# qiutang98/chord

Hardware: AMD Instinct MI355X
Metric: Gtri/s into 4K 64-bit visbuffer (higher is better)
Workload: dtype f32+u64; 1 GPU; street_4k_hzb; scene_triangles_lod0=2799616, objects=352, hzb=True, cull=flat, parallelism=single

## Files before the change

### chord_amd/csrc/kernels_raster.hip

```cpp

#include "device_layer.h"
#include "device_math.h"

#include <algorithm>
#include <cstdlib>
#include <cstring>
#include <type_traits>

namespace chord {

#define GUARD_BAND 1024.0f
#define LDS_VERTS 256
#define TILE CHORD_TILE
#define TILE_SHIFT CHORD_TILE_SHIFT
#define TPITCH (TILE + 1)
#define SMALL_AREA 256
#define TC_STRIDE CHORD_TILECOUNT_STRIDE
#define TC_BLOCKS 1u
#define TC_TICKET 2u
#ifndef CHORD_MASKED_FUSED
#define CHORD_MASKED_FUSED 1
#endif
#define TC_MASKED 3u

struct RasterParams {
    const uint32_t* count; const ChordDrawCmd* cmds;
    uint32_t cmdCap;
    uint32_t* leftCount; ChordDrawCmd* leftCmds;
    const DObjFrame* objFrame; const DObjStatic* objStatic;
    const DMeshlet* meshlets; const uint32_t* meshletData; const float* positions;
    const DMaterial* materials; const uint8_t* texAlpha; const float* texcoords;
    unsigned long long* vis;
    float* depthOut;
    float W, H; int32_t Wi, Hi;
    ShardInfo shard;
    TriRec* tris; uint32_t triCap;
    TriRecC* trisC; uint32_t triCapC;
    uint32_t* tileCount; uint32_t* tileBins; uint32_t binCap; uint32_t tilesX, tilesY;
    uint32_t* binPool; uint32_t binPoolChunks; uint32_t* binPoolCount;
    unsigned long long* binChunkTab; uint32_t binStamp; uint32_t binMaxChunks;
    unsigned long long* blockPool; uint32_t blockCap;
    uint32_t blockForce;
    ClipTri* clipTris; uint32_t clipTriCap; uint32_t pass;
    uint32_t* largeList; uint32_t largeCap;
    DeviceCounters* counters;
    uint2* tileOrder;
    unsigned long long* tileSlabs;
    uint32_t hzbFused;
    ChordHZBDesc hzbDesc;
    uint16_t* hzbMinA;
    uint16_t* hzbMinB; uint16_t* hzbMaxB;
    uint16_t* hzbExA;
    uint16_t* hzbExB;
    uint32_t* tileRange;
    unsigned long long* tileClocks;
    unsigned long long* tilePhase;
    uint32_t depthOnly, depthClamp;
    float biasConst, biasSlope;
    uint32_t clearTiles;
    uint32_t* binHint;
    uint32_t* countHint;
    uint32_t slotHot;
    uint32_t* hotTiles;
    uint32_t tileSlots;
    uint32_t tileSplitMin, tileSliceLen;
    uint2* tileOrderNext;
    uint32_t orderAll;
    uint32_t orderKept;
    uint32_t* heavyHint;
    uint32_t debug;
};
#define ABL(p, flag) (RASTER_ABLATION && ((p).debug & (flag)) != 0u)
#define DBG_NO_PIXELS   1u
#define DBG_NO_BIN      2u
#define DBG_TILE_CLOCKS 16u
#define DBG_NO_OUT      128u
#define DBG_NO_HZB      256u
#define DBG_SETUP_CLOCKS 512u
#define DBG_NO_VIS_STORE 1024u
#define DBG_NO_SPLIT    2048u
#define DBG_NO_TINY     32u
#define DBG_TILE_EXIT   64u
#define DBG_NO_ENTRY    8192u
#define DBG_NO_BATCH    16384u
#define DBG_NO_UNITS    4096u
#define DBG_SKIP_LIGHT  1048576u
#define DBG_SKIP_HEAVY  2097152u

template <typename T>
__device__ __forceinline__ T scalar_load(const T* ptr)
{
    return *reinterpret_cast<const __attribute__((address_space(4))) T*>(reinterpret_cast<uintptr_t>(ptr));
}
__device__ __forceinline__ const RasterParams* kernel_args()
{
    unsigned long long kp = (unsigned long long)__builtin_amdgcn_kernarg_segment_ptr();
    asm volatile("" : "+s"(kp));
    return reinterpret_cast<const RasterParams*>(kp);
}

__device__ __forceinline__ uint32_t mbcnt64(unsigned long long m) { return __builtin_amdgcn_mbcnt_hi((uint32_t)(m >> 32), __builtin_amdgcn_mbcnt_lo((uint32_t)m, 0u)); }
__device__ __forceinline__ int32_t bcast(int32_t v, int src) { return __builtin_amdgcn_readlane(v, src); }
__device__ __forceinline__ uint32_t bcast(uint32_t v, int src) { return (uint32_t)__builtin_amdgcn_readlane((int)v, src); }
__device__ __forceinline__ float bcast(float v, int src) { return __int_as_float(__builtin_amdgcn_readlane(__float_as_int(v), src)); }

__device__ __forceinline__ bool owns_tile(const ShardInfo& s, int32_t tx, int32_t ty)
{
    if (s.ranks <= 1) return true;
    return shard_owns_tile(s, (uint32_t)tx, (uint32_t)ty);
}
__device__ __forceinline__ bool owns_rect(const ShardInfo& s, int32_t px0, int32_t py0, int32_t px1, int32_t py1)
{
    if (s.ranks <= 1) return true;
    return shard_owns_any_tile(s, (uint32_t)px0 >> TILE_SHIFT, (uint32_t)py0 >> TILE_SHIFT, (uint32_t)px1 >> TILE_SHIFT, (uint32_t)py1 >> TILE_SHIFT);
}

__device__ __forceinline__ bool in_fast_volume_xy(const f4& h)
{
    return h.w > 0.0f && (GUARD_BAND * h.w + h.x) >= 0.0f && (GUARD_BAND * h.w - h.x) >= 0.0f &&
           (GUARD_BAND * h.w + h.y) >= 0.0f && (GUARD_BAND * h.w - h.y) >= 0.0f;
}

__device__ __forceinline__ bool in_fast_volume(const f4& h)
{
    return h.w > 0.0f && (h.w - h.z) >= 0.0f && h.z >= 0.0f &&
           (GUARD_BAND * h.w + h.x) >= 0.0f && (GUARD_BAND * h.w - h.x) >= 0.0f &&
           (GUARD_BAND * h.w + h.y) >= 0.0f && (GUARD_BAND * h.w - h.y) >= 0.0f;
}

struct TriSetup {
    int32_t X[3], Y[3];
    float d0, e1, e2, invA;
    int32_t px0, py0, px1, py1;
    int64_t area;
    int32_t s;
    uint32_t payload;
};

__device__ __forceinline__ bool narrow_extent(const TriSetup& ts)
{
    const int32_t extX = max(ts.X[0], max(ts.X[1], ts.X[2])) - min(ts.X[0], min(ts.X[1], ts.X[2]));
    const int32_t extY = max(ts.Y[0], max(ts.Y[1], ts.Y[2])) - min(ts.Y[0], min(ts.Y[1], ts.Y[2]));
    return extX <= (1 << 14) && extY <= (1 << 14);
}

__device__ __forceinline__ bool fits_compact(const TriSetup& ts)
{
    return narrow_extent(ts);
}

__device__ __forceinline__ void write_record_c(TriRecC* dst, const TriSetup& ts, const float d[3])
{
    TriRecC r;
    r.X0 = ts.X[0]; r.Y0 = ts.Y[0];
    r.dX1 = (int16_t)(ts.X[1] - ts.X[0]); r.dY1 = (int16_t)(ts.Y[1] - ts.Y[0]);
    r.dX2 = (int16_t)(ts.X[2] - ts.X[0]); r.dY2 = (int16_t)(ts.Y[2] - ts.Y[0]);
    r.d[0] = d[0]; r.d[1] = d[1]; r.d[2] = d[2];
    r.payload = ts.payload;
    *dst = r;
}

__device__ __forceinline__ bool tri_setup(TriSetup& ts, bool twoSided, int32_t Wi, int32_t Hi)
{
    const int32_t dx1 = ts.X[1] - ts.X[0], dy1 = ts.Y[1] - ts.Y[0], dx2 = ts.X[2] - ts.X[0], dy2 = ts.Y[2] - ts.Y[0];
    int64_t area2;
    const bool small = (uint32_t)(dx1 + 32767) < 65535u && (uint32_t)(dy1 + 32767) < 65535u &&
                       (uint32_t)(dx2 + 32767) < 65535u && (uint32_t)(dy2 + 32767) < 65535u;
    const bool allSmall = __ballot(!small) == 0ull;
    if (allSmall) area2 = (int64_t)(__mul24(dx1, dy2) - __mul24(dx2, dy1));
    else area2 = (int64_t)dx1 * (int64_t)dy2 - (int64_t)dx2 * (int64_t)dy1;
    if (area2 == 0) return false;
    if (!twoSided && area2 > 0) return false;
    ts.s = area2 < 0 ? -1 : 1;
    ts.area = area2 < 0 ? -area2 : area2;
    const int32_t minX = min(ts.X[0], min(ts.X[1], ts.X[2])), maxX = max(ts.X[0], max(ts.X[1], ts.X[2]));
    const int32_t minY = min(ts.Y[0], min(ts.Y[1], ts.Y[2])), maxY = max(ts.Y[0], max(ts.Y[1], ts.Y[2]));
    ts.px0 = max(0, (minX + 127) >> 8);
    ts.py0 = max(0, (minY + 127) >> 8);
    ts.px1 = min(Wi - 1, (maxX - 128) >> 8);
    ts.py1 = min(Hi - 1, (maxY - 128) >> 8);
    if (ts.px1 < ts.px0 || ts.py1 < ts.py0) return false;
    if (allSmall) ts.invA = 1.0f / (float)(int32_t)ts.area;
    else ts.invA = 1.0f / (float)(double)ts.area;
    return true;
}

__device__ __forceinline__ float depth_bias(const TriSetup& ts, const float d[3], float biasConst, float biasSlope)
{
    const int64_t s = ts.s;
    const float invA = ts.invA;
    const int64_t a1 = -s * (int64_t)(ts.Y[0] - ts.Y[2]), b1 = s * (int64_t)(ts.X[0] - ts.X[2]);
    const int64_t a2 = -s * (int64_t)(ts.Y[1] - ts.Y[0]), b2 = s * (int64_t)(ts.X[1] - ts.X[0]);
    const float e1 = d[1] - d[0], e2 = d[2] - d[0];
    const float dzdx = ((float)(double)(a1 * 256) * invA) * e1 + ((float)(double)(a2 * 256) * invA) * e2;
    const float dzdy = ((float)(double)(b1 * 256) * invA) * e1 + ((float)(double)(b2 * 256) * invA) * e2;
    const float m = fmaxf(fabsf(dzdx), fabsf(dzdy));
    const float mz = fmaxf(fabsf(d[0]), fmaxf(fabsf(d[1]), fabsf(d[2])));
    const int32_t e = (int32_t)((__float_as_uint(mz) >> 23) & 0xFFu) - 23;
    const float r = (e > 0 && e < 255) ? __uint_as_float((uint32_t)e << 23) : 0.0f;
    return biasSlope * m + biasConst * r;
}

__device__ __forceinline__ void tri_setup_from_compact(TriSetup& ts, const TriRecC& r, int32_t Wi, int32_t Hi)
{
    ts.X[0] = r.X0; ts.Y[0] = r.Y0;
    ts.X[1] = r.X0 + r.dX1; ts.Y[1] = r.Y0 + r.dY1;
    ts.X[2] = r.X0 + r.dX2; ts.Y[2] = r.Y0 + r.dY2;
    ts.payload = r.payload;
    const int32_t area2 = (int32_t)r.dX1 * (int32_t)r.dY2 - (int32_t)r.dX2 * (int32_t)r.dY1;
    ts.s = area2 < 0 ? -1 : 1;
    ts.invA = 1.0f / (float)(area2 < 0 ? -area2 : area2);
    ts.d0 = r.d[0]; ts.e1 = r.d[1] - r.d[0]; ts.e2 = r.d[2] - r.d[0];
    const int32_t minX = min(ts.X[0], min(ts.X[1], ts.X[2])), maxX = max(ts.X[0], max(ts.X[1], ts.X[2]));
    const int32_t minY = min(ts.Y[0], min(ts.Y[1], ts.Y[2])), maxY = max(ts.Y[0], max(ts.Y[1], ts.Y[2]));
    ts.px0 = max(0, (minX + 127) >> 8);
    ts.py0 = max(0, (minY + 127) >> 8);
    ts.px1 = min(Wi - 1, (maxX - 128) >> 8);
    ts.py1 = min(Hi - 1, (maxY - 128) >> 8);
    ts.area = 0;
}

__device__ __forceinline__ void tri_setup_from_record(TriSetup& ts, const TriRec& r, int32_t Wi, int32_t Hi)
{
#pragma unroll
    for (int i = 0; i < 3; i++) { ts.X[i] = r.X[i]; ts.Y[i] = r.Y[i]; }
    ts.payload = r.payload;
    ts.s = (r.twoSided & 2u) ? -1 : 1;
    ts.invA = __uint_as_float(r.pad);
    ts.d0 = r.d[0]; ts.e1 = r.d[1] - r.d[0]; ts.e2 = r.d[2] - r.d[0];
    const int32_t minX = min(ts.X[0], min(ts.X[1], ts.X[2])), maxX = max(ts.X[0], max(ts.X[1], ts.X[2]));
    const int32_t minY = min(ts.Y[0], min(ts.Y[1], ts.Y[2])), maxY = max(ts.Y[0], max(ts.Y[1], ts.Y[2]));
    ts.px0 = max(0, (minX + 127) >> 8);
    ts.py0 = max(0, (minY + 127) >> 8);
    ts.px1 = min(Wi - 1, (maxX - 128) >> 8);
    ts.py1 = min(Hi - 1, (maxY - 128) >> 8);
    ts.area = 0;
}



struct RecordEmitParams {
    DeviceCounters* counters; ClipTri* clipTris; uint32_t clipTriCap; uint32_t pass;
    TriRec* tris; uint32_t triCap; TriRecC* trisC; uint32_t triCapC; uint32_t* largeList; uint32_t largeCap;
    uint32_t* tileCount; uint32_t* tileBins; uint32_t binCap; uint32_t tilesX;
    uint32_t* binPool; uint32_t binPoolChunks; uint32_t* binPoolCount;
    unsigned long long* binChunkTab; uint32_t binStamp; uint32_t binMaxChunks;
    ShardInfo shard;
};
__device__ __forceinline__ RecordEmitParams load_record_emit_params()
{
    const RasterParams* q = kernel_args();
    RecordEmitParams e;
    e.counters = scalar_load(&q->counters); e.clipTris = scalar_load(&q->clipTris); e.clipTriCap = scalar_load(&q->clipTriCap); e.pass = scalar_load(&q->pass);
    e.tris = scalar_load(&q->tris); e.triCap = scalar_load(&q->triCap); e.trisC = scalar_load(&q->trisC); e.triCapC = scalar_load(&q->triCapC);
    e.largeList = scalar_load(&q->largeList); e.largeCap = scalar_load(&q->largeCap);
    e.tileCount = scalar_load(&q->tileCount); e.tileBins = scalar_load(&q->tileBins); e.binCap = scalar_load(&q->binCap); e.tilesX = scalar_load(&q->tilesX);
    e.binPool = scalar_load(&q->binPool); e.binPoolChunks = scalar_load(&q->binPoolChunks); e.binPoolCount = scalar_load(&q->binPoolCount);
    e.binChunkTab = scalar_load(&q->binChunkTab); e.binStamp = scalar_load(&q->binStamp); e.binMaxChunks = scalar_load(&q->binMaxChunks);
    e.shard.ranks = scalar_load(&q->shard.ranks); e.shard.rank = scalar_load(&q->shard.rank); e.shard.slotsPerRank = 0u; e.shard.tilesX = 0u;
    e.shard.ownedRows = scalar_load(&q->shard.ownedRows); e.shard.tileSlot = nullptr;
    return e;
}

struct BinElect { int leader; uint32_t rank, group; };

__device__ __forceinline__ BinElect wave_bin_elect(bool has, uint32_t tile, uint32_t lane)
{
    BinElect e; e.leader = 0; e.rank = 0; e.group = 0;
    unsigned long long todo = __ballot(has);
    const unsigned long long lt = (1ull << lane) - 1ull;
    while (todo) {
        const int l = __ffsll((long long)todo) - 1;
        const uint32_t k = bcast(tile, l);
        const unsigned long long same = __ballot(has && tile == k);
        if (has && tile == k) { e.leader = l; e.rank = (uint32_t)__popcll(same & lt); e.group = (uint32_t)__popcll(same); }
        todo &= ~same;
    }
    return e;
}

__device__ __forceinline__ uint32_t bin_capacity(const RasterParams& p) { return p.binCap + p.binMaxChunks * CHORD_BIN_CHUNK; }

template <class P>
__device__ __forceinline__ void bin_alloc(const P& p, uint32_t tile, uint32_t slot)
{
#ifdef EXP_NO_CHUNKS
    return;
#endif
    if (slot < p.binCap) return;
    const uint32_t o = slot - p.binCap, j = o >> CHORD_BIN_CHUNK_SHIFT;
    if (j >= p.binMaxChunks || (o & (CHORD_BIN_CHUNK - 1u)) != 0u) return;
    uint32_t id = atomicAdd(p.binPoolCount, 1u);
    if (id >= p.binPoolChunks) { id = CHORD_BIN_CHUNK_INVALID; atomicOr(&p.counters->overflow, 1u); }
    __hip_atomic_store(p.binChunkTab + (__umul24(tile, p.binMaxChunks) + j), ((unsigned long long)p.binStamp << 32) | id,
                       __ATOMIC_RELAXED, __HIP_MEMORY_SCOPE_AGENT);
}

template <class P>
__device__ __forceinline__ void bin_put(const P& p, uint32_t tile, uint32_t slot, uint32_t gi)
{
#ifdef EXP_NO_CHUNKS
    slot &= p.binCap - 1u;
#endif
    if (slot < p.binCap) { p.tileBins[__umul24(tile, p.binCap) + slot] = gi; return; }
    const uint32_t o = slot - p.binCap, j = o >> CHORD_BIN_CHUNK_SHIFT;
    if (j >= p.binMaxChunks) { atomicOr(&p.counters->overflow, 1u); return; }
    const unsigned long long* ent = p.binChunkTab + (__umul24(tile, p.binMaxChunks) + j);
    const unsigned long long stamp = (unsigned long long)p.binStamp << 32;
    unsigned long long e = 0;
    uint32_t spins = 0;
    for (;;) {
        e = __hip_atomic_load(ent, __ATOMIC_RELAXED, __HIP_MEMORY_SCOPE_AGENT);
        if ((e & 0xFFFFFFFF00000000ull) == stamp) break;
        if (++spins > (1u << 20)) { atomicOr(&p.counters->overflow, 4u); return; }
        __builtin_amdgcn_s_sleep(4);
    }
    const uint32_t id = (uint32_t)e;
    if (id != CHORD_BIN_CHUNK_INVALID) p.binPool[((size_t)id << CHORD_BIN_CHUNK_SHIFT) + (o & (CHORD_BIN_CHUNK - 1u))] = gi;
}

__device__ __forceinline__ void bin_store(const RasterParams& p, uint32_t tile, uint32_t slot, uint32_t gi)
{
    bin_alloc(p, tile, slot);
    bin_put(p, tile, slot, gi);
}

struct BinTicket {
    uint32_t tileA[4], tileB[4], slotA[4], slotB[4];
    uint32_t has;
    uint32_t eA[4], eB[4];
};

template <class P>
__device__ __forceinline__ void wave_bin_issue(const P& p, bool emitA, const TriSetup& tsA, bool emitB, const TriSetup& tsB,
                                               uint32_t lane, BinTicket& k, const bool masked = false)
{
    auto tile_of = [&](const TriSetup& ts, int r, bool emit, uint32_t& tile) -> bool {
        const int32_t tx0 = ts.px0 >> TILE_SHIFT, tx1 = ts.px1 >> TILE_SHIFT, ty0 = ts.py0 >> TILE_SHIFT, ty1 = ts.py1 >> TILE_SHIFT;
        const int32_t tx = (r & 1) ? tx1 : tx0, ty = (r & 2) ? ty1 : ty0;
        bool has = emit && !((r & 1) && tx1 == tx0) && !((r & 2) && ty1 == ty0);
        if (has) has = owns_tile(p.shard, tx, ty);
        tile = has ? __umul24((uint32_t)ty, p.tilesX) + (uint32_t)tx : 0u;
        return has;
    };
    k.has = 0u;
#pragma unroll
    for (int r = 0; r < 4; r++) {
        k.slotA[r] = 0u; k.slotB[r] = 0u;
        if (tile_of(tsA, r, emitA, k.tileA[r])) k.has |= 1u << r;
        if (tile_of(tsB, r, emitB, k.tileB[r])) k.has |= 16u << r;
    }
#pragma unroll
    for (int r = 0; r < 4; r++) {
        const BinElect a = wave_bin_elect((k.has & (1u << r)) != 0u, k.tileA[r], lane);
        const BinElect b = wave_bin_elect((k.has & (16u << r)) != 0u, k.tileB[r], lane);
        k.eA[r] = (uint32_t)a.leader | a.rank << 8; k.eB[r] = (uint32_t)b.leader | b.rank << 8;
        if ((k.has & (1u << r)) && (int)lane == a.leader) k.slotA[r] = atomicAdd(&p.tileCount[(size_t)k.tileA[r] * TC_STRIDE], a.group);
        if ((k.has & (16u << r)) && (int)lane == b.leader) k.slotB[r] = atomicAdd(&p.tileCount[(size_t)k.tileB[r] * TC_STRIDE], b.group);
    }
    if (masked) {
#pragma unroll
        for (int r = 0; r < 4; r++) {
            if ((k.has & (1u << r)) && lane == (k.eA[r] & 0xFFu)) p.tileCount[(size_t)k.tileA[r] * TC_STRIDE + TC_MASKED] = 1u;
            if ((k.has & (16u << r)) && lane == (k.eB[r] & 0xFFu)) p.tileCount[(size_t)k.tileB[r] * TC_STRIDE + TC_MASKED] = 1u;
        }
    }
}

template <class P>
__device__ __forceinline__ void wave_bin_commit(const P& p, BinTicket& k, bool okA, uint32_t giA, bool okB, uint32_t giB)
{
#pragma unroll
    for (int r = 0; r < 4; r++) {
        k.slotA[r] = __shfl(k.slotA[r], (int)(k.eA[r] & 0xFFu), 64) + (k.eA[r] >> 8);
        k.slotB[r] = __shfl(k.slotB[r], (int)(k.eB[r] & 0xFFu), 64) + (k.eB[r] >> 8);
    }
    if (k.has) {
#pragma unroll
        for (int r = 0; r < 4; r++) {
            if (k.has & (1u << r)) bin_alloc(p, k.tileA[r], k.slotA[r]);
            if (k.has & (16u << r)) bin_alloc(p, k.tileB[r], k.slotB[r]);
        }
    }
#pragma unroll
    for (int r = 0; r < 4; r++) {
        if (okA && (k.has & (1u << r))) bin_put(p, k.tileA[r], k.slotA[r], giA);
        if (okB && (k.has & (16u << r))) bin_put(p, k.tileB[r], k.slotB[r], giB);
    }
}

__device__ __forceinline__ bool touches_many_tiles(const TriSetup& ts)
{
    return ((ts.px1 >> TILE_SHIFT) - (ts.px0 >> TILE_SHIFT)) > 1 || ((ts.py1 >> TILE_SHIFT) - (ts.py0 >> TILE_SHIFT)) > 1;
}

__device__ __forceinline__ void write_record(TriRec* dst, const TriSetup& ts, const float d[3], bool twoSided, bool masked = false)
{
    TriRec r;
#pragma unroll
    for (int i = 0; i < 3; i++) { r.X[i] = ts.X[i]; r.Y[i] = ts.Y[i]; r.d[i] = d[i]; }
    r.payload = ts.payload;
    r.twoSided = (twoSided ? 1u : 0u) | (ts.s < 0 ? 2u : 0u) | (masked ? 4u : 0u);
    r.pad = __float_as_uint(ts.invA);
    *dst = r;
}

__device__ __forceinline__ bool filter_is_linear(uint32_t f)
{
    return f == CHORD_FILTER_LINEAR || f == CHORD_FILTER_LINEAR_MIPMAP_NEAREST || f == CHORD_FILTER_LINEAR_MIPMAP_LINEAR;
}

__device__ __forceinline__ uint32_t mask_level_filter(const DMaterial& m, int64_t absArea2, const float u[3], const float v[3])
{
    uint32_t level = 0u;
    bool linear = filter_is_linear(m.magFilter);
    if (m.texOffset != 0xFFFFFFFFu) {
        const float texels = (float)m.texWidth * (float)m.texHeight;
        const float auv = fabsf((u[1] - u[0]) * (v[2] - v[0]) - (u[2] - u[0]) * (v[1] - v[0])) * texels;
        const float apx = (float)(double)absArea2 * (1.0f / 65536.0f);
        const float ratio = auv / apx;
        if (ratio >= 1.0f) {
            const int32_t e = (int32_t)((__float_as_uint(ratio) >> 23) & 0xFFu) - 127;
            level = min((uint32_t)(e >> 1), m.texMips - 1u);
            linear = filter_is_linear(m.minFilter);
        }
    }
    return level | (linear ? 256u : 0u);
}

__device__ __forceinline__ void write_mask_ext(TriRec* slot, const DMaterial* mp, uint32_t material, int64_t absArea2,
                                               const float u[3], const float v[3], const float w[3])
{
    DMaterial m;
    m.texOffset = mp->texOffset; m.texWidth = mp->texWidth; m.texHeight = mp->texHeight; m.texMips = mp->texMips;
    m.minFilter = mp->minFilter; m.magFilter = mp->magFilter; m.wrapS = mp->wrapS; m.wrapT = mp->wrapT;
    m.alphaFactor = mp->alphaFactor; m.alphaCutOff = mp->alphaCutOff;
    TriRecMaskExt e;
#pragma unroll
    for (int i = 0; i < 3; i++) { e.iw[i] = 1.0f / w[i]; e.uw[i] = u[i] * e.iw[i]; e.vw[i] = v[i] * e.iw[i]; }
    e.levelFilter = mask_level_filter(m, absArea2, u, v);
    (void)material;
    const uint32_t level = e.levelFilter & 0xFFu;
    e.levelBase = 0xFFFFFFFFu; e.dims = 0u; e.magicS = e.biasS = e.magicT = e.biasT = 0u;
    if (m.texOffset != 0xFFFFFFFFu) {
        const DMatLevel L = mp->levels[level];
        e.levelBase = L.base; e.dims = L.dims;
        e.magicS = L.magicS; e.biasS = L.biasS; e.magicT = L.magicT; e.biasT = L.biasT;
    }
    e.wraps = (m.wrapS & 0xFFFFu) | m.wrapT << 16;
    e.alphaFactor = m.alphaFactor; e.alphaCutOff = m.alphaCutOff;
    uint4* dst = reinterpret_cast<uint4*>(slot);
    const uint4* src = reinterpret_cast<const uint4*>(&e);
    dst[0] = src[0]; dst[1] = src[1]; dst[2] = src[2]; dst[3] = src[3];
    reinterpret_cast<uint32_t*>(slot)[16] = e.biasS; reinterpret_cast<uint32_t*>(slot)[17] = e.magicT; reinterpret_cast<uint32_t*>(slot)[18] = e.biasT;
}

#ifndef EXP_MASKED
#define EXP_MASKED 0
#endif
__device__ __forceinline__ int32_t period_mod(int32_t i, int32_t period, uint32_t magic, uint32_t bias)
{
    if ((EXP_MASKED & 4) || magic == 0u) return i & (period - 1);
    const uint32_t iu = (uint32_t)i + bias;
    uint32_t r = iu - __umulhi(iu, magic) * (uint32_t)period;
    if (r >= (uint32_t)period) r -= (uint32_t)period;
    return (int32_t)r;
}
__device__ __forceinline__ int32_t wrap_index(int32_t i, int32_t n, uint32_t mode, uint32_t magic, uint32_t bias)
{
    if (mode == CHORD_WRAP_CLAMP_TO_EDGE) return i < 0 ? 0 : (i > n - 1 ? n - 1 : i);
    if (mode == CHORD_WRAP_MIRRORED_REPEAT) {
        const int32_t m = period_mod(i, 2 * n, magic, bias);
        return m < n ? m : 2 * n - 1 - m;
    }
    return period_mod(i, n, magic, bias);
}

__device__ __forceinline__ void wrap_pair(int32_t i, int32_t n, uint32_t mode, uint32_t magic, uint32_t bias, int32_t& w0, int32_t& w1)
{
    if (mode == CHORD_WRAP_CLAMP_TO_EDGE) {
        w0 = i < 0 ? 0 : (i > n - 1 ? n - 1 : i);
        w1 = i + 1 < 0 ? 0 : (i + 1 > n - 1 ? n - 1 : i + 1);
        return;
    }
    const bool mirror = mode == CHORD_WRAP_MIRRORED_REPEAT;
    const int32_t period = mirror ? 2 * n : n;
    const int32_t m = period_mod(i, period, magic, bias);
    const int32_t m1 = m + 1 == period ? 0 : m + 1;
    w0 = mirror ? (m < n ? m : 2 * n - 1 - m) : m;
    w1 = mirror ? (m1 < n ? m1 : 2 * n - 1 - m1) : m1;
}

__device__ __forceinline__ int32_t texel_floor(float x)
{
    if (!(fabsf(x) < 1.0e9f)) return 0;
    return (int32_t)floorf(x);
}

struct AlphaLevel {
    const uint8_t* base;
    int32_t W, H;
    float fW, fH;
    uint32_t wrapS, wrapT;
    uint32_t magicS, biasS, magicT, biasT;
    bool linear;
};
__device__ __forceinline__ AlphaLevel alpha_level(const uint8_t* __restrict__ texAlpha, const TriRecMaskExt& e)
{
    const uint32_t levelBase = e.levelBase, dims = e.dims;
    AlphaLevel a;
    a.base = nullptr; a.W = 1; a.H = 1; a.fW = 1.0f; a.fH = 1.0f; a.wrapS = e.wraps & 0xFFFFu; a.wrapT = e.wraps >> 16; a.linear = (e.levelFilter & 256u) != 0u;
    a.magicS = e.magicS; a.biasS = e.biasS; a.magicT = e.magicT; a.biasT = e.biasT;
    if (levelBase == 0xFFFFFFFFu) return a;
    a.W = (int32_t)(dims & 0xFFFFu) + 1; a.H = (int32_t)(dims >> 16) + 1;
    a.fW = (float)a.W; a.fH = (float)a.H;
    a.base = texAlpha + levelBase;
    return a;
}
__device__ __forceinline__ float sample_alpha(const AlphaLevel& t, float u, float v)
{
    if (!t.base) return 1.0f;
    if (EXP_MASKED & 1) return 1.0f;
    if (!t.linear || (EXP_MASKED & 2)) {
        const int32_t ix = wrap_index(texel_floor(u * t.fW), t.W, t.wrapS, t.magicS, t.biasS), iy = wrap_index(texel_floor(v * t.fH), t.H, t.wrapT, t.magicT, t.biasT);
        return (float)t.base[iy * t.W + ix] * (1.0f / 255.0f);
    }
    const float x = u * t.fW - 0.5f, y = v * t.fH - 0.5f;
    const int32_t x0 = texel_floor(x), y0 = texel_floor(y);
    float fx = x - (float)x0, fy = y - (float)y0;
    if (!(fabsf(x) < 1.0e9f)) fx = 0.0f;
    if (!(fabsf(y) < 1.0e9f)) fy = 0.0f;
    int32_t ix0, ix1, iy0, iy1;
    wrap_pair(x0, t.W, t.wrapS, t.magicS, t.biasS, ix0, ix1);
    wrap_pair(y0, t.H, t.wrapT, t.magicT, t.biasT, iy0, iy1);
    const float a00 = (float)t.base[iy0 * t.W + ix0] * (1.0f / 255.0f), a10 = (float)t.base[iy0 * t.W + ix1] * (1.0f / 255.0f);
    const float a01 = (float)t.base[iy1 * t.W + ix0] * (1.0f / 255.0f), a11 = (float)t.base[iy1 * t.W + ix1] * (1.0f / 255.0f);
    const float top = a00 + (a10 - a00) * fx, bot = a01 + (a11 - a01) * fx;
    return top + (bot - top) * fy;
}

__device__ __forceinline__ void setup_emit_mask_ext(const RasterParams& p, TriRec* slot, uint32_t triWord, const float uv[6],
                                                 const float* lW, uint32_t material, int64_t absArea2)
{
    float u[3], v[3], w[3];
#pragma unroll
    for (int i = 0; i < 3; i++) {
        u[i] = uv[2 * i]; v[i] = uv[2 * i + 1];
        w[i] = lW[(triWord >> (8 * i)) & 0xFFu];
    }
    write_mask_ext(slot, &p.materials[material], material, absArea2, u, v, w);
}

template <int PITCH>
__device__ __forceinline__ void tile_raster_narrow(unsigned long long* tile, const TriSetup& ts, int32_t ox, int32_t oy,
                                                   int32_t x0, int32_t y0, int32_t x1, int32_t y1, bool noPixels, const bool clampZ);

__device__ __forceinline__ void wave_min2_max2(int32_t& a, int32_t& b, int32_t& c, int32_t& d)
{
#define DPP_STEP(ctrl)                                                \
    "v_min_i32_dpp %0, %0, %0 " ctrl "\n\t"                           \
    "v_min_i32_dpp %1, %1, %1 " ctrl "\n\t"                           \
    "v_max_i32_dpp %2, %2, %2 " ctrl "\n\t"                           \
    "v_max_i32_dpp %3, %3, %3 " ctrl "\n\t"
    asm volatile("s_nop 1\n\t"
                 DPP_STEP("quad_perm:[1,0,3,2] row_mask:0xf bank_mask:0xf")
                 DPP_STEP("quad_perm:[2,3,0,1] row_mask:0xf bank_mask:0xf")
                 DPP_STEP("row_ror:4 row_mask:0xf bank_mask:0xf")
                 DPP_STEP("row_ror:8 row_mask:0xf bank_mask:0xf")
                 DPP_STEP("row_bcast:15 row_mask:0xa bank_mask:0xf")
                 DPP_STEP("row_bcast:31 row_mask:0xc bank_mask:0xf")
                 "s_nop 0"
                 : "+v"(a), "+v"(b), "+v"(c), "+v"(d));
#undef DPP_STEP
    a = __builtin_amdgcn_readlane(a, 63); b = __builtin_amdgcn_readlane(b, 63);
    c = __builtin_amdgcn_readlane(c, 63); d = __builtin_amdgcn_readlane(d, 63);
}

__device__ __forceinline__ void wave_sum2(uint32_t& a, uint32_t& b)
{
#define DPP_STEP(ctrl)                                                \
    "v_add_u32_dpp %0, %0, %0 " ctrl "\n\t"                           \
    "v_add_u32_dpp %1, %1, %1 " ctrl "\n\t"
    asm volatile("s_nop 1\n\t"
                 DPP_STEP("quad_perm:[1,0,3,2] row_mask:0xf bank_mask:0xf") "s_nop 0\n\t"
                 DPP_STEP("quad_perm:[2,3,0,1] row_mask:0xf bank_mask:0xf") "s_nop 0\n\t"
                 DPP_STEP("row_ror:4 row_mask:0xf bank_mask:0xf") "s_nop 0\n\t"
                 DPP_STEP("row_ror:8 row_mask:0xf bank_mask:0xf") "s_nop 0\n\t"
                 DPP_STEP("row_bcast:15 row_mask:0xa bank_mask:0xf") "s_nop 0\n\t"
                 DPP_STEP("row_bcast:31 row_mask:0xc bank_mask:0xf")
                 "s_nop 0"
                 : "+v"(a), "+v"(b));
#undef DPP_STEP
    a = (uint32_t)__builtin_amdgcn_readlane((int)a, 63); b = (uint32_t)__builtin_amdgcn_readlane((int)b, 63);
}

enum { K_NONE = 0, K_EMIT = 1, K_CLIP = 2 };
#define WIN CHORD_BLOCK_WIN
#define DBG_NO_BLOCKS 32768u
#define DBG_FORCE_BLOCKS 65536u
#define DBG_FORCE_HOT 262144u

template <bool MASKED>
__device__ __forceinline__ void raster_setup_body(const RasterParams& p, const ChordDrawCmd* __restrict__ cmds, const uint32_t count, float (*sVert)[4][LDS_VERTS],
                                                  const uint32_t firstCmd0, const uint32_t firstCmd1, const uint32_t firstCmd2, const bool firstCmdValid)
{
    const uint32_t lane = threadIdx.x & 63u, wave = threadIdx.x >> 6;
    float* lX = sVert[0][wave]; float* lY = sVert[1][wave]; float* lW = sVert[2][wave];
    float* lU = sVert[3][wave]; float* lV = sVert[4][wave]; float* lD = sVert[5][wave];

    const uint32_t listShard = (blockIdx.x * 4u + wave) % CHORD_LIST_SHARDS;

    struct Header {
        uint32_t objectId, meshletId, slot, V, T, dataOffset, vertexBase, matFlags;
        bool twoSided;
    };
    auto header_of = [&](uint32_t objectId, uint32_t meshletId, uint32_t slot) -> Header {
        Header h;
        h.objectId = objectId; h.meshletId = meshletId; h.slot = slot;
        const RasterParams* q = kernel_args();
        const DMeshlet* __restrict__ mm = &scalar_load(&q->meshlets)[h.meshletId];
        const uint32_t vt = scalar_load(&mm->vertexTriangleCount);
        h.V = vt & 0xFFu; h.T = (vt >> 8) & 0xFFu;
        h.dataOffset = scalar_load(&mm->dataOffset);
        h.vertexBase = scalar_load(&mm->vertexBase);
        h.matFlags = scalar_load(&scalar_load(&q->objStatic)[h.objectId].matFlags);
        h.twoSided = (h.matFlags & CHORD_MATFLAG_TWO_SIDED) != 0u;
        if (CHORD_MATFLAG_ALPHA(h.matFlags) >= CHORD_ALPHA_BLEND) h.T = 0u;
        return h;
    };
    auto load_header = [&](uint32_t i) -> Header {
        const uint32_t k = __builtin_amdgcn_readfirstlane(min(i, count - 1u));
        const uint32_t* __restrict__ cw = reinterpret_cast<const uint32_t*>(cmds + k);
        return header_of(scalar_load(cw), scalar_load(cw + 1), scalar_load(cw + 2));
    };
    auto mvp_of = [&](uint32_t objectId) -> Mat4 {
        Mat4 m;
        const float* __restrict__ mv = scalar_load(&kernel_args()->objFrame)[objectId].mvp;
#pragma unroll
        for (int r = 0; r < 4; r++)
#pragma unroll
            for (int cc = 0; cc < 4; cc++) m.r[r][cc] = scalar_load(mv + r * 4 + cc);
        return m;
    };
    const uint32_t stride = gridDim.x * 4u;
    uint32_t c = blockIdx.x * 4u + wave;
    if (c >= count) return;
    Header hdr = firstCmdValid ? header_of(firstCmd0, firstCmd1, firstCmd2) : load_header(c);
    Header hdrN = load_header(c + stride);
    Mat4 mvpNext = mvp_of(hdr.objectId);
    uint32_t t0 = 0, t1 = 0;
    float pax, pay, paz, pbx, pby, pbz;
    {
        const uint32_t* __restrict__ md = scalar_load(&kernel_args()->meshletData);
        const float* __restrict__ ps = scalar_load(&kernel_args()->positions);
        const uint32_t ia = md[hdr.dataOffset + min(lane, max(hdr.V, 1u) - 1u)] + hdr.vertexBase;
        const uint32_t ib = md[hdr.dataOffset + min(lane + 64u, max(hdr.V, 1u) - 1u)] + hdr.vertexBase;
        if (lane < hdr.T) t0 = md[hdr.dataOffset + hdr.V + lane];
        if (lane + 64u < hdr.T) t1 = md[hdr.dataOffset + hdr.V + 64u + lane];
        const float* __restrict__ pa = ps + (size_t)(ia * 3u);
        const float* __restrict__ pb = ps + (size_t)(ib * 3u);
        pax = pa[0]; pay = pa[1]; paz = pa[2]; pbx = pb[0]; pby = pb[1]; pbz = pb[2];
    }
    const bool sprof = RASTER_PROFILE && (p.debug & DBG_SETUP_CLOCKS) != 0;
    unsigned long long sph[5] = {0, 0, 0, 0, 0}, stp = sprof ? wall_clock64() : 0ull;
#define SPHASE(i) do { if (sprof) { const unsigned long long tn = wall_clock64(); sph[i] += tn - stp; stp = tn; } } while (0)
    const uint32_t laneTop = lane;
    for (; c < count; c += stride) {
        uint32_t lane = laneTop;
        asm volatile("" : "+v"(lane));
        const uint32_t slot = hdr.slot, V = hdr.V, T = hdr.T, dataOffset = hdr.dataOffset, vertexBase = hdr.vertexBase;
        const bool twoSided = hdr.twoSided || p.depthOnly != 0u;
        const bool masked = MASKED && CHORD_MATFLAG_ALPHA(hdr.matFlags) == CHORD_ALPHA_MASK;
        const Mat4 mvp = mvpNext;
        const uint32_t triWord[2] = {t0, t1};

        if (sprof) { volatile uint32_t sink = V + T; (void)sink; }
        SPHASE(0);
        bool notFast = false;
        auto vertex = [&](uint32_t i, float x, float y, float z) {
            const f4 h = mul_mv(mvp, x, y, z, 1.0f);
            const float aw = fabsf(h.w);
            lX[i] = h.x; lY[i] = h.y; lW[i] = h.w;
            lU[i] = h.x / aw * 0.5f + 0.5f;
            lV[i] = h.y / aw * -0.5f + 0.5f;
            const bool fast = p.depthClamp ? in_fast_volume_xy(h) : in_fast_volume(h);
            lD[i] = fast ? h.z / h.w : __builtin_nanf("");
            notFast = notFast || !fast;
        };
        if (lane < V) vertex(lane, pax, pay, paz);
        if (lane + 64u < V) vertex(lane + 64u, pbx, pby, pbz);
        for (uint32_t i = lane + 128u; i < V; i += 64u) {
            const float* __restrict__ pp = scalar_load(&kernel_args()->positions) + (size_t)(scalar_load(&kernel_args()->meshletData)[dataOffset + i] + vertexBase) * 3;
            vertex(i, pp[0], pp[1], pp[2]);
        }
        const bool allFast = __ballot(notFast) == 0ull;
        __builtin_amdgcn_fence(__ATOMIC_RELEASE, "wavefront");
        __builtin_amdgcn_wave_barrier();
        __builtin_amdgcn_fence(__ATOMIC_ACQUIRE, "wavefront");
        SPHASE(1);
        const uint32_t* __restrict__ mdN = scalar_load(&kernel_args()->meshletData);
        const uint32_t nia = mdN[hdrN.dataOffset + min(lane, max(hdrN.V, 1u) - 1u)] + hdrN.vertexBase;
        const uint32_t nib = mdN[hdrN.dataOffset + min(lane + 64u, max(hdrN.V, 1u) - 1u)] + hdrN.vertexBase;
        const uint32_t nt0 = lane < hdrN.T ? mdN[hdrN.dataOffset + hdrN.V + lane] : 0u;
        const uint32_t nt1 = lane + 64u < hdrN.T ? mdN[hdrN.dataOffset + hdrN.V + 64u + lane] : 0u;

        float uvA[6] = {0.0f, 0.0f, 0.0f, 0.0f, 0.0f, 0.0f}, uvB[6] = {0.0f, 0.0f, 0.0f, 0.0f, 0.0f, 0.0f};
        if (MASKED && masked && scalar_load(&kernel_args()->texcoords) != nullptr) {
            const float* __restrict__ tc = scalar_load(&kernel_args()->texcoords);
            const uint32_t* __restrict__ mdT = scalar_load(&kernel_args()->meshletData);
#pragma unroll
            for (int i = 0; i < 3; i++) {
                if (lane < T) { const size_t vi = (size_t)(mdT[dataOffset + ((t0 >> (8 * i)) & 0xFFu)] + vertexBase) * 2; uvA[2 * i] = tc[vi]; uvA[2 * i + 1] = tc[vi + 1]; }
                if (lane + 64u < T) { const size_t vi = (size_t)(mdT[dataOffset + ((t1 >> (8 * i)) & 0xFFu)] + vertexBase) * 2; uvB[2 * i] = tc[vi]; uvB[2 * i + 1] = tc[vi + 1]; }
            }
        }
        int kindA = K_NONE, kindB = K_NONE;
        TriSetup tsA, tsB;
        float dA[3] = {0.0f, 0.0f, 0.0f}, dB[3] = {0.0f, 0.0f, 0.0f};
        tsA.px0 = tsA.py0 = tsA.px1 = tsA.py1 = 0; tsB.px0 = tsB.py0 = tsB.px1 = tsB.py1 = 0;
#pragma unroll
        for (int half = 0; half < 2; half++) {
            const uint32_t t = (uint32_t)half * 64u + lane;
            int kind = K_NONE;
            TriSetup ts;
            ts.px0 = ts.py0 = ts.px1 = ts.py1 = 0;
            float d[3] = {0.0f, 0.0f, 0.0f};
            if (t < T) {
                const uint32_t packedIdx = triWord[half];
                const uint32_t i0 = packedIdx & 0xFFu, i1 = (packedIdx >> 8) & 0xFFu, i2 = (packedIdx >> 16) & 0xFFu;
                const float x0 = lX[i0], y0 = lY[i0], w0 = lW[i0];
                const float x1 = lX[i1], y1 = lY[i1], w1 = lW[i1];
                const float x2 = lX[i2], y2 = lY[i2], w2 = lW[i2];
                bool culled = false;
                if (!twoSided) {
                    const float det = (x0 * (y1 * w2 - w1 * y2) - y0 * (x1 * w2 - w1 * x2)) + w0 * (x1 * y2 - y1 * x2);
                    culled = det <= 0.0f;
                }
                culled = culled || (w0 <= 0.0f && w1 <= 0.0f && w2 <= 0.0f);
                const float u0 = lU[i0], v0 = lV[i0], u1 = lU[i1], v1 = lV[i1], u2 = lU[i2], v2 = lV[i2];
                const float maxU = fmaxf(u0, fmaxf(u1, u2)), maxV = fmaxf(v0, fmaxf(v1, v2));
                const float minU = fminf(u0, fminf(u1, u2)), minV = fminf(v0, fminf(v1, v2));
                culled = culled || ((minU >= 1.0f || minV >= 1.0f) || (maxU <= 0.0f || maxV <= 0.0f));
                culled = culled || (rintf(minU * p.W) == rintf(maxU * p.W) || rintf(minV * p.H) == rintf(maxV * p.H));
                if (!culled) {
                    d[0] = lD[i0]; d[1] = lD[i1]; d[2] = lD[i2];
                    ts.payload = p.depthOnly ? 0u : encode_triangle_instance(t, slot);
                    if (!allFast && (d[0] != d[0] || d[1] != d[1] || d[2] != d[2])) {
                        kind = K_CLIP;
                    } else {
                        ts.X[0] = (int32_t)rintf((u0 * p.W) * 256.0f); ts.Y[0] = (int32_t)rintf((v0 * p.H) * 256.0f);
                        ts.X[1] = (int32_t)rintf((u1 * p.W) * 256.0f); ts.Y[1] = (int32_t)rintf((v1 * p.H) * 256.0f);
                        ts.X[2] = (int32_t)rintf((u2 * p.W) * 256.0f); ts.Y[2] = (int32_t)rintf((v2 * p.H) * 256.0f);
                        if (tri_setup(ts, twoSided, p.Wi, p.Hi) && owns_rect(p.shard, ts.px0, ts.py0, ts.px1, ts.py1)) {
                            kind = K_EMIT;
                            if (p.biasConst != 0.0f || p.biasSlope != 0.0f) { const float o = depth_bias(ts, d, p.biasConst, p.biasSlope); d[0] += o; d[1] += o; d[2] += o; }
                        }
                    }
                }
            }
            if (ABL(p, DBG_NO_BIN)) kind = K_NONE;
            if (half == 0) { kindA = kind; tsA = ts; dA[0] = d[0]; dA[1] = d[1]; dA[2] = d[2]; }
            else           { kindB = kind; tsB = ts; dB[0] = d[0]; dB[1] = d[1]; dB[2] = d[2]; }
        }
        SPHASE(2);
        const float* __restrict__ psN = scalar_load(&kernel_args()->positions);
        const float* __restrict__ npa = psN + (size_t)(nia * 3u);
        const float* __restrict__ npb = psN + (size_t)(nib * 3u);
        const float nax = npa[0], nay = npa[1], naz = npa[2], nbx = npb[0], nby = npb[1], nbz = npb[2];
        {
            const unsigned long long lt = (1ull << lane) - 1ull;
            const unsigned long long cmA = __ballot(kindA == K_CLIP), cmB = __ballot(kindB == K_CLIP);
            const unsigned long long emA = __ballot(kindA == K_EMIT), emB = __ballot(kindB == K_EMIT);
            const bool cpA = kindA == K_EMIT && !masked && fits_compact(tsA), cpB = kindB == K_EMIT && !masked && fits_compact(tsB);
            const uint32_t wSlots = masked ? 1u + CHORD_MASK_EXT_SLOTS : 1u;
            const unsigned long long ecA = __ballot(cpA), ecB = __ballot(cpB);
            const unsigned long long ewA = emA & ~ecA, ewB = emB & ~ecB;
            const bool lgA = kindA == K_EMIT && touches_many_tiles(tsA), lgB = kindB == K_EMIT && touches_many_tiles(tsB);
            const unsigned long long lmA = __ballot(lgA), lmB = __ballot(lgB);
            const uint32_t nClip = (uint32_t)(__popcll(cmA) + __popcll(cmB));
            const uint32_t nEc = (uint32_t)(__popcll(ecA) + __popcll(ecB)), nEw = (uint32_t)(__popcll(ewA) + __popcll(ewB));
            const uint32_t nLg = (uint32_t)(__popcll(lmA) + __popcll(lmB));
            {
            const RecordEmitParams e = load_record_emit_params();
            uint32_t cbase = 0, ebaseC = 0, ebaseW = 0, lbase = 0;
            if (lane == 0) {
                if (nClip) cbase = atomicAdd(&e.counters->clipTriCount[p.pass], nClip);
                if (nEc) ebaseC = atomicAdd(&e.counters->triCountC[listShard * CHORD_SHARD_STRIDE], nEc);
                if (nEw) ebaseW = atomicAdd(&e.counters->triCount[listShard * CHORD_SHARD_STRIDE], nEw * wSlots);
                if (nLg) lbase = atomicAdd(&e.counters->largeCount[p.pass][listShard * CHORD_SHARD_STRIDE], nLg);
            }
            BinTicket ticket;
            if (emA | emB) wave_bin_issue(e, kindA == K_EMIT && !lgA, tsA, kindB == K_EMIT && !lgB, tsB, lane, ticket, MASKED && masked);
            cbase = bcast(cbase, 0); ebaseC = bcast(ebaseC, 0); ebaseW = bcast(ebaseW, 0); lbase = bcast(lbase, 0);
            SPHASE(3);
            mvpNext = mvp_of(hdrN.objectId);
            if (kindA == K_CLIP) {
                const uint32_t k = cbase + (uint32_t)__popcll(cmA & lt);
                if (k < e.clipTriCap) { ClipTri ct; ct.objectId = hdr.objectId; ct.meshletId = hdr.meshletId; ct.slot = hdr.slot; ct.tri = lane; e.clipTris[k] = ct; }
                else atomicOr(&e.counters->overflow, 2u);
            }
            if (kindB == K_CLIP) {
                const uint32_t k = cbase + (uint32_t)__popcll(cmA) + (uint32_t)__popcll(cmB & lt);
                if (k < e.clipTriCap) { ClipTri ct; ct.objectId = hdr.objectId; ct.meshletId = hdr.meshletId; ct.slot = hdr.slot; ct.tri = lane + 64u; e.clipTris[k] = ct; }
                else atomicOr(&e.counters->overflow, 2u);
            }
            uint32_t giA = 0, giB = 0;
            bool okA = false, okB = false;
            if (cpA) {
                const uint32_t li = ebaseC + (uint32_t)__popcll(ecA & lt);
                if (li < e.triCapC) { giA = listShard * e.triCapC + li; write_record_c(&e.trisC[giA], tsA, dA); okA = true; }
                else atomicOr(&e.counters->overflow, 1u);
            } else if (kindA == K_EMIT) {
                const uint32_t li = ebaseW + wSlots * (uint32_t)__popcll(ewA & lt);
                if (li + wSlots <= e.triCap) {
                    giA = listShard * e.triCap + li; write_record(&e.tris[giA], tsA, dA, twoSided, masked);
                    if (MASKED && masked) setup_emit_mask_ext(p, &e.tris[giA + 1u], triWord[0], uvA, lW, CHORD_MATFLAG_MATERIAL(hdr.matFlags), tsA.area);
                    giA |= (MASKED && masked) ? CHORD_REC_MASKED : CHORD_REC_WIDE; okA = true;
                } else atomicOr(&e.counters->overflow, 1u);
            }
            if (cpB) {
                const uint32_t li = ebaseC + (uint32_t)__popcll(ecA) + (uint32_t)__popcll(ecB & lt);
                if (li < e.triCapC) { giB = listShard * e.triCapC + li; write_record_c(&e.trisC[giB], tsB, dB); okB = true; }
                else atomicOr(&e.counters->overflow, 1u);
            } else if (kindB == K_EMIT) {
                const uint32_t li = ebaseW + wSlots * ((uint32_t)__popcll(ewA) + (uint32_t)__popcll(ewB & lt));
                if (li + wSlots <= e.triCap) {
                    giB = listShard * e.triCap + li; write_record(&e.tris[giB], tsB, dB, twoSided, masked);
                    if (MASKED && masked) setup_emit_mask_ext(p, &e.tris[giB + 1u], triWord[1], uvB, lW, CHORD_MATFLAG_MATERIAL(hdr.matFlags), tsB.area);
                    giB |= (MASKED && masked) ? CHORD_REC_MASKED : CHORD_REC_WIDE; okB = true;
                } else atomicOr(&e.counters->overflow, 1u);
            }
            if (emA | emB) wave_bin_commit(e, ticket, okA, giA, okB, giB);
            if (lgA && okA) {
                const uint32_t k = lbase + (uint32_t)__popcll(lmA & lt);
                if (k < e.largeCap) e.largeList[(size_t)listShard * e.largeCap + k] = giA & CHORD_REC_WIDE_INDEX; else atomicOr(&e.counters->overflow, 1u);
            }
            if (lgB && okB) {
                const uint32_t k = lbase + (uint32_t)__popcll(lmA) + (uint32_t)__popcll(lmB & lt);
                if (k < e.largeCap) e.largeList[(size_t)listShard * e.largeCap + k] = giB & CHORD_REC_WIDE_INDEX; else atomicOr(&e.counters->overflow, 1u);
            }
            }
        }
        __builtin_amdgcn_fence(__ATOMIC_RELEASE, "wavefront");
        __builtin_amdgcn_wave_barrier();
        hdr = hdrN;
        hdrN = load_header(c + 2u * stride);
        t0 = nt0; t1 = nt1;
        pax = nax; pay = nay; paz = naz; pbx = nbx; pby = nby; pbz = nbz;
        SPHASE(4);
    }
    if (sprof && lane == 0u) {
        const uint32_t w = blockIdx.x * 4u + wave;
        if (w < CHORD_MAX_TILES * 8u / 5u) for (int i = 0; i < 5; i++) p.tilePhase[(size_t)w * 5u + i] = sph[i];
    }
#undef SPHASE
}

struct SetupHeader { uint32_t objectId, meshletId, slot, V, T, dataOffset, vertexBase, matFlags; };

struct BlockEmitParams {
    uint32_t* tileCount; uint32_t* tileBins; uint32_t binCap;
    uint32_t* binPool; uint32_t binPoolChunks; uint32_t* binPoolCount;
    unsigned long long* binChunkTab; uint32_t binStamp; uint32_t binMaxChunks;
    unsigned long long* blockPool; uint32_t blockCap;
    DeviceCounters* counters;
};
__device__ __forceinline__ BlockEmitParams load_block_emit_params()
{
    const RasterParams* q = kernel_args();
    BlockEmitParams e;
    e.tileCount = scalar_load(&q->tileCount); e.tileBins = scalar_load(&q->tileBins); e.binCap = scalar_load(&q->binCap);
    e.binPool = scalar_load(&q->binPool); e.binPoolChunks = scalar_load(&q->binPoolChunks); e.binPoolCount = scalar_load(&q->binPoolCount);
    e.binChunkTab = scalar_load(&q->binChunkTab); e.binStamp = scalar_load(&q->binStamp); e.binMaxChunks = scalar_load(&q->binMaxChunks);
    e.blockPool = scalar_load(&q->blockPool); e.blockCap = scalar_load(&q->blockCap);
    e.counters = scalar_load(&q->counters);
    return e;
}

#define WAVE_LDS_SYNC() do { __builtin_amdgcn_fence(__ATOMIC_RELEASE, "wavefront"); __builtin_amdgcn_wave_barrier(); __builtin_amdgcn_fence(__ATOMIC_ACQUIRE, "wavefront"); } while (0)

__device__ __forceinline__ int classify_triangle(const RasterParams& p, uint32_t t, uint32_t T, uint32_t packedIdx, bool twoSided, bool allFast,
                                                 const float* lX, const float* lY, const float* lW, const float* lU, const float* lV, const float* lD,
                                                 const int32_t* lSX, const int32_t* lSY, uint32_t& boxX, uint32_t& boxY, bool& narrow)
{
    boxX = 0u; boxY = 0u; narrow = false;
    if (t >= T) return K_NONE;
    const uint32_t i0 = packedIdx & 0xFFu, i1 = (packedIdx >> 8) & 0xFFu, i2 = (packedIdx >> 16) & 0xFFu;
    const float w0 = lW[i0], w1 = lW[i1], w2 = lW[i2];
    bool culled = false;
    if (!twoSided) {
        const float x0 = lX[i0], y0 = lY[i0], x1 = lX[i1], y1 = lY[i1], x2 = lX[i2], y2 = lY[i2];
        const float det = (x0 * (y1 * w2 - w1 * y2) - y0 * (x1 * w2 - w1 * x2)) + w0 * (x1 * y2 - y1 * x2);
        culled = det <= 0.0f;
    }
    culled = culled || (w0 <= 0.0f && w1 <= 0.0f && w2 <= 0.0f);
    const float u0 = lU[i0], v0 = lV[i0], u1 = lU[i1], v1 = lV[i1], u2 = lU[i2], v2 = lV[i2];
    const float maxU = fmaxf(u0, fmaxf(u1, u2)), maxV = fmaxf(v0, fmaxf(v1, v2));
    const float minU = fminf(u0, fminf(u1, u2)), minV = fminf(v0, fminf(v1, v2));
    culled = culled || ((minU >= 1.0f || minV >= 1.0f) || (maxU <= 0.0f || maxV <= 0.0f));
    culled = culled || (rintf(minU * p.W) == rintf(maxU * p.W) || rintf(minV * p.H) == rintf(maxV * p.H));
    if (culled) return K_NONE;
    if (!allFast) { const float d0 = lD[i0], d1 = lD[i1], d2 = lD[i2]; if (d0 != d0 || d1 != d1 || d2 != d2) return K_CLIP; }
    const int32_t X0 = lSX[i0], Y0 = lSY[i0], X1 = lSX[i1], Y1 = lSY[i1], X2 = lSX[i2], Y2 = lSY[i2];
    const int32_t minX = min(X0, min(X1, X2)), maxX = max(X0, max(X1, X2));
    const int32_t minY = min(Y0, min(Y1, Y2)), maxY = max(Y0, max(Y1, Y2));
    if (maxX - minX > (1 << 14) || maxY - minY > (1 << 14)) return K_EMIT;
    narrow = true;
    const int32_t area2 = __mul24(X1 - X0, Y2 - Y0) - __mul24(X2 - X0, Y1 - Y0);
    if (area2 == 0 || (!twoSided && area2 > 0)) return K_NONE;
    const int32_t px0 = max(0, (minX + 127) >> 8), py0 = max(0, (minY + 127) >> 8);
    const int32_t px1 = min(p.Wi - 1, (maxX - 128) >> 8), py1 = min(p.Hi - 1, (maxY - 128) >> 8);
    if (px1 < px0 || py1 < py0) return K_NONE;
    boxX = (uint32_t)px0 | ((uint32_t)px1 << 16); boxY = (uint32_t)py0 | ((uint32_t)py1 << 16);
    return K_EMIT;
}

__device__ __forceinline__ void resolve_entry(const RasterParams& p, uint32_t entry, uint32_t boxX, uint32_t boxY, uint32_t slot,
                                              const int32_t* lSX, const int32_t* lSY, const float* lD, unsigned long long* win,
                                              int32_t bx0, int32_t by0)
{
    const uint32_t i0 = entry & 0xFFu, i1 = (entry >> 8) & 0xFFu, i2 = (entry >> 16) & 0xFFu, t = entry >> 24;
    TriSetup ts;
    ts.X[0] = lSX[i0]; ts.Y[0] = lSY[i0];
    ts.X[1] = lSX[i1]; ts.Y[1] = lSY[i1];
    ts.X[2] = lSX[i2]; ts.Y[2] = lSY[i2];
    const int32_t dx1 = ts.X[1] - ts.X[0], dy1 = ts.Y[1] - ts.Y[0], dx2 = ts.X[2] - ts.X[0], dy2 = ts.Y[2] - ts.Y[0];
    const int32_t area2 = __mul24(dx1, dy2) - __mul24(dx2, dy1);
    const int32_t area = area2 < 0 ? -area2 : area2;
    ts.s = area2 < 0 ? -1 : 1;
    ts.area = (int64_t)area;
    ts.invA = 1.0f / (float)area;
    ts.px0 = (int32_t)(boxX & 0xFFFFu); ts.px1 = (int32_t)(boxX >> 16);
    ts.py0 = (int32_t)(boxY & 0xFFFFu); ts.py1 = (int32_t)(boxY >> 16);
    float d[3] = {lD[i0], lD[i1], lD[i2]};
    if (p.biasConst != 0.0f || p.biasSlope != 0.0f) { const float o = depth_bias(ts, d, p.biasConst, p.biasSlope); d[0] += o; d[1] += o; d[2] += o; }
    ts.payload = p.depthOnly ? 0u : encode_triangle_instance(t, slot);
    ts.d0 = d[0]; ts.e1 = d[1] - d[0]; ts.e2 = d[2] - d[0];
    if (p.depthClamp != 0u) tile_raster_narrow<WIN>(win, ts, bx0, by0, ts.px0, ts.py0, ts.px1, ts.py1, false, true);
    else tile_raster_narrow<WIN>(win, ts, bx0, by0, ts.px0, ts.py0, ts.px1, ts.py1, false, false);
}

#define SLOT_CACHE 32u
#define SLOT_HOT 65536u
#ifndef SLOT_AHEAD
#define SLOT_AHEAD 8u
#endif
#ifndef SLOT_AHEAD_VERY_HOT
#define SLOT_AHEAD_VERY_HOT 32u
#endif
#define SLOT_VERY_HOT 262144u
struct SlotCache { uint32_t key[SLOT_CACHE], next[SLOT_CACHE], end[SLOT_CACHE]; uint32_t pend; };

#ifndef BLOCKS_LDS_VERTS
#define BLOCKS_LDS_VERTS 128
#endif
template <bool HOT>
__device__ __forceinline__ void raster_setup_blocks_body(const RasterParams& p, const uint32_t count, float (*sVert)[4][BLOCKS_LDS_VERTS], int32_t (*sSnap)[4][BLOCKS_LDS_VERTS],
                                                         unsigned long long (*sWin)[WIN * WIN], SlotCache* slotCaches)
{
    const uint32_t lane = threadIdx.x & 63u, wave = threadIdx.x >> 6;
    SlotCache& sc = slotCaches[HOT ? wave : 0u];
    if (HOT && lane < SLOT_CACHE) { sc.key[lane] = 0u; sc.next[lane] = 0u; sc.end[lane] = 0u; }
    if (HOT) {
        const uint32_t* __restrict__ hl = scalar_load(&kernel_args()->hotTiles);
        WAVE_LDS_SYNC();
        if (hl) {
            const uint32_t nHot = min(hl[0], (uint32_t)CHORD_HOT_TILES);
            if (lane < nHot) {
                const uint32_t e = hl[1u + lane], tile = e & 0xFFFu, ci = tile & (SLOT_CACHE - 1u);
                const uint32_t pos = (e >> 31) ? SLOT_VERY_HOT : 0u;
                sc.key[ci] = tile + 1u; sc.next[ci] = pos; sc.end[ci] = pos;
            }
        }
        WAVE_LDS_SYNC();
    }
    float* lX = sVert[0][wave]; float* lY = sVert[1][wave]; float* lW = sVert[2][wave];
    float* lU = sVert[3][wave]; float* lV = sVert[4][wave]; float* lD = sVert[5][wave];
    int32_t* lSX = sSnap[0][wave]; int32_t* lSY = sSnap[1][wave];
    unsigned long long* win = sWin[wave];
    const uint32_t listShard = (blockIdx.x * 4u + wave) % CHORD_LIST_SHARDS;

    auto kq = [&]() -> const RasterParams* { return kernel_args(); };
    auto header_at = [&](uint32_t i) -> SetupHeader {
        const uint32_t k = __builtin_amdgcn_readfirstlane(min(i, count - 1u));
        SetupHeader h;
        const RasterParams* q = kq();
        const uint32_t* __restrict__ cw = reinterpret_cast<const uint32_t*>(scalar_load(&q->cmds) + k);
        h.objectId = scalar_load(cw); h.meshletId = scalar_load(cw + 1); h.slot = scalar_load(cw + 2);
        const DMeshlet* __restrict__ mm = &scalar_load(&q->meshlets)[h.meshletId];
        const uint32_t vt = scalar_load(&mm->vertexTriangleCount);
        h.V = vt & 0xFFu; h.T = (vt >> 8) & 0xFFu;
        h.dataOffset = scalar_load(&mm->dataOffset);
        h.vertexBase = scalar_load(&mm->vertexBase);
        h.matFlags = scalar_load(&scalar_load(&q->objStatic)[h.objectId].matFlags);
        if (CHORD_MATFLAG_ALPHA(h.matFlags) >= CHORD_ALPHA_BLEND) h.T = 0u;
        return h;
    };
    auto mvp_of = [&](uint32_t objectId) -> Mat4 {
        Mat4 m;
        const float* __restrict__ mv = scalar_load(&kq()->objFrame)[objectId].mvp;
#pragma unroll
        for (int r = 0; r < 4; r++)
#pragma unroll
            for (int cc = 0; cc < 4; cc++) m.r[r][cc] = scalar_load(mv + r * 4 + cc);
        return m;
    };
    const uint32_t stride = gridDim.x * 4u;
    uint32_t c = blockIdx.x * 4u + wave;
    if (c >= count) return;
    SetupHeader hdr = header_at(c);
    SetupHeader hdrN = header_at(c + stride);
    uint32_t t0 = 0, t1 = 0;
    float pax, pay, paz, pbx, pby, pbz;
    {
        const uint32_t* __restrict__ md = scalar_load(&kq()->meshletData);
        const float* __restrict__ ps = scalar_load(&kq()->positions);
        const uint32_t ia = md[hdr.dataOffset + min(lane, max(hdr.V, 1u) - 1u)] + hdr.vertexBase;
        const uint32_t ib = md[hdr.dataOffset + min(lane + 64u, max(hdr.V, 1u) - 1u)] + hdr.vertexBase;
        if (lane < hdr.T) t0 = md[hdr.dataOffset + hdr.V + lane];
        if (lane + 64u < hdr.T) t1 = md[hdr.dataOffset + hdr.V + 64u + lane];
        const float* __restrict__ pa = ps + (size_t)(ia * 3u);
        const float* __restrict__ pb = ps + (size_t)(ib * 3u);
        pax = pa[0]; pay = pa[1]; paz = pa[2]; pbx = pb[0]; pby = pb[1]; pbz = pb[2];
    }
    const bool sprof = RASTER_PROFILE && (p.debug & DBG_SETUP_CLOCKS) != 0;
    unsigned long long sph[5] = {0, 0, 0, 0, 0}, stp = sprof ? wall_clock64() : 0ull;
#define SPHASE(i) do { if (sprof) { const unsigned long long tn = wall_clock64(); sph[i] += tn - stp; stp = tn; } } while (0)
    for (; c < count; c += stride) {
        const uint32_t V = hdr.V, T = hdr.T, dataOffset = hdr.dataOffset, vertexBase = hdr.vertexBase;
        const bool twoSided = (hdr.matFlags & CHORD_MATFLAG_TWO_SIDED) != 0u || p.depthOnly != 0u;
        const bool masked = CHORD_MATFLAG_ALPHA(hdr.matFlags) == CHORD_ALPHA_MASK;
        if (sprof) { volatile uint32_t sink = V + T; (void)sink; }
        SPHASE(0);
        const bool tooBig = V > (uint32_t)BLOCKS_LDS_VERTS;
        (void)dataOffset; (void)vertexBase;
        bool notFast = false;
        if (!tooBig) {
            const Mat4 mvp = mvp_of(hdr.objectId);
            auto vertex = [&](uint32_t i, float x, float y, float z) {
                const f4 h = mul_mv(mvp, x, y, z, 1.0f);
                const float aw = fabsf(h.w);
                lX[i] = h.x; lY[i] = h.y; lW[i] = h.w;
                const float u = h.x / aw * 0.5f + 0.5f, v = h.y / aw * -0.5f + 0.5f;
                lU[i] = u; lV[i] = v;
                lSX[i] = (int32_t)rintf((u * p.W) * 256.0f); lSY[i] = (int32_t)rintf((v * p.H) * 256.0f);
                const bool fast = p.depthClamp ? in_fast_volume_xy(h) : in_fast_volume(h);
                lD[i] = fast ? h.z / h.w : __builtin_nanf("");
                notFast = notFast || !fast;
            };
            if (lane < V) vertex(lane, pax, pay, paz);
            if (lane + 64u < V) vertex(lane + 64u, pbx, pby, pbz);
#if BLOCKS_LDS_VERTS > 128
            for (uint32_t i = lane + 128u; i < V; i += 64u) {
                const float* __restrict__ pp = scalar_load(&kq()->positions) + (size_t)(scalar_load(&kq()->meshletData)[dataOffset + i] + vertexBase) * 3;
                vertex(i, pp[0], pp[1], pp[2]);
            }
#endif
        }
        const bool allFast = __ballot(notFast) == 0ull;
        WAVE_LDS_SYNC();
        SPHASE(1);
        const uint32_t* __restrict__ md = scalar_load(&kq()->meshletData);
        const uint32_t nia = md[hdrN.dataOffset + min(lane, max(hdrN.V, 1u) - 1u)] + hdrN.vertexBase;
        const uint32_t nib = md[hdrN.dataOffset + min(lane + 64u, max(hdrN.V, 1u) - 1u)] + hdrN.vertexBase;
        const uint32_t nt0 = lane < hdrN.T ? md[hdrN.dataOffset + hdrN.V + lane] : 0u;
        const uint32_t nt1 = lane + 64u < hdrN.T ? md[hdrN.dataOffset + hdrN.V + 64u + lane] : 0u;

        uint32_t bxA, byA, bxB, byB;
        bool nwA, nwB;
        int kindA = classify_triangle(p, lane, tooBig ? 0u : T, t0, twoSided, allFast, lX, lY, lW, lU, lV, lD, lSX, lSY, bxA, byA, nwA);
        int kindB = classify_triangle(p, lane + 64u, tooBig ? 0u : T, t1, twoSided, allFast, lX, lY, lW, lU, lV, lD, lSX, lSY, bxB, byB, nwB);
        if (ABL(p, DBG_NO_BIN)) { kindA = K_NONE; kindB = K_NONE; }
        SPHASE(2);
        const float* __restrict__ ps = scalar_load(&kq()->positions);
        const float* __restrict__ npa = ps + (size_t)(nia * 3u);
        const float* __restrict__ npb = ps + (size_t)(nib * 3u);
        const float nax = npa[0], nay = npa[1], naz = npa[2], nbx = npb[0], nby = npb[1], nbz = npb[2];

        const bool eA = kindA == K_EMIT, eB = kindB == K_EMIT;
        const unsigned long long emA = __ballot(eA), emB = __ballot(eB);
        const unsigned long long bad = __ballot(kindA == K_CLIP || kindB == K_CLIP || (eA && !nwA) || (eB && !nwB)) | (tooBig && T != 0u ? 1ull : 0ull);
        bool blocksDone = false;
        if (!masked && (emA | emB) != 0ull && bad == 0ull) {
            int32_t bx0 = min(eA ? (int32_t)(bxA & 0xFFFFu) : 0x7FFF, eB ? (int32_t)(bxB & 0xFFFFu) : 0x7FFF);
            int32_t by0 = min(eA ? (int32_t)(byA & 0xFFFFu) : 0x7FFF, eB ? (int32_t)(byB & 0xFFFFu) : 0x7FFF);
            int32_t bx1 = max(eA ? (int32_t)(bxA >> 16) : -1, eB ? (int32_t)(bxB >> 16) : -1);
            int32_t by1 = max(eA ? (int32_t)(byA >> 16) : -1, eB ? (int32_t)(byB >> 16) : -1);
            if (__ballot(bx1 - bx0 >= WIN || by1 - by0 >= WIN) == 0ull) {
                wave_min2_max2(bx0, by0, bx1, by1);
                const int32_t bw = bx1 - bx0 + 1, bh = by1 - by0 + 1;
                const uint32_t nE = (uint32_t)(__popcll(emA) + __popcll(emB));
                if (bw <= WIN && bh <= WIN && (uint32_t)(bw * bh + 8) * 8u <= nE * 36u) {
                    blocksDone = true;
                    const int32_t tx0 = bx0 >> TILE_SHIFT, tx1 = bx1 >> TILE_SHIFT, ty0 = by0 >> TILE_SHIFT, ty1 = by1 >> TILE_SHIFT;
                    const uint32_t r = lane & 3u;
                    const bool sx = (r & 1u) != 0u, sy = (r & 2u) != 0u;
                    const int32_t rx0 = sx ? tx1 << TILE_SHIFT : bx0, rx1 = (sx || tx1 == tx0) ? bx1 : (tx0 << TILE_SHIFT) + TILE - 1;
                    const int32_t ry0 = sy ? ty1 << TILE_SHIFT : by0, ry1 = (sy || ty1 == ty0) ? by1 : (ty0 << TILE_SHIFT) + TILE - 1;
                    const uint32_t rw = (uint32_t)(rx1 - rx0 + 1), rh = (uint32_t)(ry1 - ry0 + 1);
                    const bool has = lane < 4u && !(sx && tx1 == tx0) && !(sy && ty1 == ty0) && owns_tile(p.shard, sx ? tx1 : tx0, sy ? ty1 : ty0);
                    const uint32_t hasMask = (uint32_t)__ballot(has) & 15u;
                    const uint32_t gran = has ? (rw * rh + 2u) >> 1 : 0u;
                    const uint32_t g0 = bcast(gran, 0), g1 = bcast(gran, 1), g2 = bcast(gran, 2), g3 = bcast(gran, 3);
                    const uint32_t before = (r > 0u ? g0 : 0u) + (r > 1u ? g1 : 0u) + (r > 2u ? g2 : 0u), G = g0 + g1 + g2 + g3;
                    const uint32_t tile = __umul24((uint32_t)(sy ? ty1 : ty0), p.tilesX) + (uint32_t)(sx ? tx1 : tx0);
                    uint32_t gbase = 0, slot = 0;
                    const BlockEmitParams e = load_block_emit_params();
                    {
                        uint32_t ahead = 1u;
                        if (HOT) {
                            const uint32_t ci = tile & (SLOT_CACHE - 1u);
                            if (lane == 0u && has && sc.key[ci] == tile + 1u) {
                                const uint32_t nx = sc.next[ci];
                                if (nx < sc.end[ci]) { slot = nx; sc.next[ci] = nx + 1u; ahead = 0u; }
                                else ahead = nx >= SLOT_VERY_HOT ? SLOT_AHEAD_VERY_HOT : SLOT_AHEAD;
                            }
                            if (lane == 0u) sc.pend = ahead;
                        }
                        if (lane == 0u && G) gbase = atomicAdd(&e.counters->blockGranules[listShard * CHORD_SHARD_STRIDE], G);
                        if (has && ahead) slot = (uint32_t)atomicAdd(reinterpret_cast<unsigned long long*>(&e.tileCount[(size_t)tile * TC_STRIDE]), (unsigned long long)ahead * 0x100000001ull);
                    }
                    uint32_t* lList = reinterpret_cast<uint32_t*>(lX);
                    uint32_t* lBoxX = reinterpret_cast<uint32_t*>(lY);
                    uint32_t* lBoxY = reinterpret_cast<uint32_t*>(lW);
                    const uint32_t nA = (uint32_t)__popcll(emA);
                    WAVE_LDS_SYNC();
                    if (eA) { const uint32_t k = mbcnt64(emA); lList[k] = (t0 & 0xFFFFFFu) | lane << 24; lBoxX[k] = bxA; lBoxY[k] = byA; }
                    if (eB) { const uint32_t k = nA + mbcnt64(emB); lList[k] = (t1 & 0xFFFFFFu) | (lane + 64u) << 24; lBoxX[k] = bxB; lBoxY[k] = byB; }
#pragma unroll
                    for (int k = 0; k < WIN * WIN / 64; k++) win[lane + 64u * k] = 0ull;
                    WAVE_LDS_SYNC();
                    const bool anyPart = hasMask != 0u;
                    if (anyPart) {
                        if (lane < nE) resolve_entry(p, lList[lane], lBoxX[lane], lBoxY[lane], hdr.slot, lSX, lSY, lD, win, bx0, by0);
                        if (nE > 64u) {
                            __builtin_amdgcn_sched_barrier(0);
                            if (lane + 64u < nE) resolve_entry(p, lList[lane + 64u], lBoxX[lane + 64u], lBoxY[lane + 64u], hdr.slot, lSX, lSY, lD, win, bx0, by0);
                        }
                    }
                    WAVE_LDS_SYNC();
                    SPHASE(3);
                    gbase = bcast(gbase, 0);
                    const bool fits = gbase + G <= e.blockCap;
                    if (!fits && lane == 0u) atomicOr(&e.counters->overflow, 1u);
                    const uint32_t off = listShard * e.blockCap + gbase + before;
                    uint32_t drew = 1u;
                    if (HOT) {
                        if (lane == 0u) drew = sc.pend;
                        if (lane == 0u && has && drew) {
                            const uint32_t ci = tile & (SLOT_CACHE - 1u);
                            if (drew > 1u) {
                                sc.next[ci] = slot + 1u; sc.end[ci] = slot + drew;
                                for (uint32_t k = 1u; k < drew; k++) bin_alloc(e, tile, slot + k);
                            } else if (slot >= scalar_load(&kq()->slotHot) && (sc.key[ci] == 0u || sc.next[ci] >= sc.end[ci])) {
                                sc.key[ci] = tile + 1u; sc.next[ci] = 0u; sc.end[ci] = 0u;
                            }
                        }
                    }
                    if (has && drew) bin_alloc(e, tile, slot);
                    if (has && fits) bin_put(e, tile, slot, CHORD_REC_BLOCK | off);
                    if (fits) {
                        for (uint32_t q = 0; q < 4u; q++) {
                            if (!((hasMask >> q) & 1u)) continue;
                            const uint32_t qoff = bcast(off, (int)q), qw = bcast(rw, (int)q), qh = bcast(rh, (int)q);
                            const uint32_t qx = (uint32_t)bcast(rx0 - bx0, (int)q), qy = (uint32_t)bcast(ry0 - by0, (int)q);
                            const uint32_t qlx = (uint32_t)bcast(rx0 & (TILE - 1), (int)q), qly = (uint32_t)bcast(ry0 & (TILE - 1), (int)q);
                            const uint32_t n = qw * qh, gq = (n + 2u) >> 1;
                            const uint32_t rcp = (uint32_t)ceilf(65536.0f * __builtin_amdgcn_rcpf((float)qw));
                            const unsigned long long header = (unsigned long long)(qlx | qly << 6 | (qw - 1u) << 12 | (qh - 1u) << 16) | ((unsigned long long)rcp << 32);
                            ulonglong2* dst = reinterpret_cast<ulonglong2*>(e.blockPool + (size_t)qoff * 2u);
                            for (uint32_t g = lane; g < gq; g += 64u) {
                                const uint32_t j1 = 2u * g, j0 = g == 0u ? 0u : j1 - 1u;
                                const uint32_t row0 = __umul24(j0, rcp) >> 16, row1 = __umul24(j1, rcp) >> 16;
                                const unsigned long long w0 = g == 0u ? header : win[(qy + row0) * WIN + qx + (j0 - __umul24(row0, qw))];
                                const unsigned long long w1 = j1 < n ? win[(qy + row1) * WIN + qx + (j1 - __umul24(row1, qw))] : 0ull;
                                dst[g] = make_ulonglong2(w0, w1);
                            }
                        }
                    }
                }
            }
        }
        if (!blocksDone && ((emA | emB) != 0ull || bad != 0ull)) {
            if (lane == 0u) {
                const uint32_t k = atomicAdd(scalar_load(&kq()->leftCount), 1u);
                ChordDrawCmd cmd; cmd.objectId = hdr.objectId; cmd.meshletId = hdr.meshletId; cmd.slot = hdr.slot;
                scalar_load(&kq()->leftCmds)[k] = cmd;
            }
            SPHASE(3);
        }
        __builtin_amdgcn_fence(__ATOMIC_RELEASE, "wavefront");
        __builtin_amdgcn_wave_barrier();
        hdr = hdrN;
        hdrN = header_at(c + 2u * stride);
        t0 = nt0; t1 = nt1;
        pax = nax; pay = nay; paz = naz; pbx = nbx; pby = nby; pbz = nbz;
        SPHASE(4);
    }
    if (HOT) WAVE_LDS_SYNC();
    if (HOT && lane < SLOT_CACHE && sc.key[lane] != 0u && sc.next[lane] < sc.end[lane]) {
        const BlockEmitParams e = load_block_emit_params();
        for (uint32_t k = sc.next[lane]; k < sc.end[lane]; k++) bin_put(e, sc.key[lane] - 1u, k, 0xFFFFFFFFu);
    }
    if (sprof && lane == 0u) {
        const uint32_t w = blockIdx.x * 4u + wave;
        if (w < CHORD_MAX_TILES * 8u / 5u) for (int i = 0; i < 5; i++) p.tilePhase[(size_t)w * 5u + i] = sph[i];
    }
#undef SPHASE
}

__device__ __forceinline__ bool launch_is_dense(const RasterParams& p, uint32_t count)
{
    const unsigned long long pixels = (unsigned long long)p.Wi * (unsigned long long)p.Hi / (p.shard.ranks > 1u ? p.shard.ranks : 1u);
    return p.blockCap != 0u && p.leftCmds != nullptr && (p.blockForce != 0u || (unsigned long long)count * 16ull >= pixels);
}

#ifndef SETUP_MIN_WAVES
#define SETUP_MIN_WAVES 5
#endif
#ifndef BLOCKS_MIN_WAVES
#define BLOCKS_MIN_WAVES 6
#endif
#ifndef SETUP_MASKED_WAVES
#define SETUP_MASKED_WAVES 4
#endif
template <bool MASKED>
__global__ __launch_bounds__(256, MASKED ? SETUP_MASKED_WAVES : SETUP_MIN_WAVES) void raster_setup_kernel(RasterParams p)
{
    __shared__ float sVert[6][4][LDS_VERTS];
    const uint32_t c0 = __builtin_amdgcn_readfirstlane(min(blockIdx.x * 4u + (threadIdx.x >> 6), p.cmdCap - 1u));
    const uint32_t* __restrict__ cw = reinterpret_cast<const uint32_t*>(p.cmds + c0);
    const uint32_t f0 = scalar_load(cw), f1 = scalar_load(cw + 1), f2 = scalar_load(cw + 2);
    uint32_t count = *p.count;
    const ChordDrawCmd* cmds = p.cmds;
    bool firstValid = true;
    if (launch_is_dense(p, count)) { count = *p.leftCount; cmds = p.leftCmds; firstValid = false; }
    raster_setup_body<MASKED>(p, cmds, count, sVert, f0, f1, f2, firstValid);
}

template <bool HOT>
__global__ __launch_bounds__(256, BLOCKS_MIN_WAVES) void raster_setup_blocks_kernel(RasterParams p)
{
    __shared__ float sVert[6][4][BLOCKS_LDS_VERTS];
    __shared__ int32_t sSnap[2][4][BLOCKS_LDS_VERTS];
    __shared__ unsigned long long sWin[4][WIN * WIN];
    __shared__ SlotCache sSlots[HOT ? 4 : 1];
    const uint32_t count = *p.count;
    if (!launch_is_dense(p, count)) return;
    raster_setup_blocks_body<HOT>(p, count, sVert, sSnap, sWin, sSlots);
}

__device__ void bin_record_tiles(const RasterParams& p, const TriSetup& ts, uint32_t gi)
{
    const int ea[3] = {1, 2, 0}, eb[3] = {2, 0, 1};
    const int32_t tx0 = ts.px0 >> TILE_SHIFT, tx1 = ts.px1 >> TILE_SHIFT;
    const int32_t ty0 = ts.py0 >> TILE_SHIFT, ty1 = ts.py1 >> TILE_SHIFT;
    for (int32_t ty = ty0; ty <= ty1; ty++)
        for (int32_t tx = tx0; tx <= tx1; tx++) {
            const int32_t rx0 = max(ts.px0, tx << TILE_SHIFT), rx1 = min(ts.px1, (tx << TILE_SHIFT) + TILE - 1);
            const int32_t ry0 = max(ts.py0, ty << TILE_SHIFT), ry1 = min(ts.py1, (ty << TILE_SHIFT) + TILE - 1);
            bool hit = owns_tile(p.shard, tx, ty);
#pragma unroll
            for (int i = 0; i < 3; i++) {
                const int64_t dxe = (int64_t)(ts.X[eb[i]] - ts.X[ea[i]]), dye = (int64_t)(ts.Y[eb[i]] - ts.Y[ea[i]]);
                const int64_t a = -(int64_t)ts.s * dye, b = (int64_t)ts.s * dxe;
                const int64_t bias = (a > 0 || (a == 0 && b > 0)) ? 0 : -1;
                const int64_t cx = (int64_t)(a > 0 ? rx1 : rx0) * 256 + 128, cy = (int64_t)(b > 0 ? ry1 : ry0) * 256 + 128;
                hit = hit && !((int64_t)ts.s * (dxe * (cy - ts.Y[ea[i]]) - dye * (cx - ts.X[ea[i]])) + bias < 0);
            }
            if (!hit) continue;
            const uint32_t tile = (uint32_t)ty * p.tilesX + (uint32_t)tx;
            const uint32_t slot = atomicAdd(&p.tileCount[(size_t)tile * TC_STRIDE], 1u);
            bin_store(p, tile, slot, gi);
            if ((gi & 0xE0000000u) == CHORD_REC_MASKED) p.tileCount[(size_t)tile * TC_STRIDE + TC_MASKED] = 1u;
        }
}

__device__ __forceinline__ float clip_dist(const f4& v, int k)
{
    switch (k) {
    case 0: return v.w - v.z;
    case 1: return v.z;
    case 2: return GUARD_BAND * v.w + v.x;
    case 3: return GUARD_BAND * v.w - v.x;
    case 4: return GUARD_BAND * v.w + v.y;
    default: return GUARD_BAND * v.w - v.y;
    }
}

__device__ __forceinline__ f4 clip_intersect(const f4& in, const f4& out, float din, float dout)
{
    const float t = din / (din - dout);
    f4 r;
    r.x = in.x + (out.x - in.x) * t;
    r.y = in.y + (out.y - in.y) * t;
    r.z = in.z + (out.z - in.z) * t;
    r.w = in.w + (out.w - in.w) * t;
    return r;
}

#define CLIP_MAXV 10
#define CLIP_THREADS 64u
template <uint32_t STRIDE>
struct ClipLds {
    float4* poly; float* pu; float* pv; int32_t* px; int32_t* py; float* pd; uint32_t tl;
    __device__ __forceinline__ float4& P(int bf, int i) const { return poly[((uint32_t)bf * CLIP_MAXV + (uint32_t)i) * STRIDE + tl]; }
    __device__ __forceinline__ float& U(int bf, int i) const { return pu[((uint32_t)bf * CLIP_MAXV + (uint32_t)i) * STRIDE + tl]; }
    __device__ __forceinline__ float& V(int bf, int i) const { return pv[((uint32_t)bf * CLIP_MAXV + (uint32_t)i) * STRIDE + tl]; }
    __device__ __forceinline__ int32_t& X(int i) const { return px[(uint32_t)i * STRIDE + tl]; }
    __device__ __forceinline__ int32_t& Y(int i) const { return py[(uint32_t)i * STRIDE + tl]; }
    __device__ __forceinline__ float& D(int i) const { return pd[(uint32_t)i * STRIDE + tl]; }
};

template <uint32_t STRIDE>
__device__ __forceinline__ int clip_triangle(const RasterParams& p, const ClipLds<STRIDE>& L, const DMeshlet& m, uint32_t V, uint32_t tri,
                                             const Mat4& mvp, bool masked, int& cur)
{
    const uint32_t packedIdx = p.meshletData[m.dataOffset + V + tri];
    for (int i = 0; i < 3; i++) {
        const uint32_t li = (packedIdx >> (8 * i)) & 0xFFu;
        const uint32_t vi = p.meshletData[m.dataOffset + li] + m.vertexBase;
        const float* pos = p.positions + (size_t)vi * 3;
        const f4 h = mul_mv(mvp, pos[0], pos[1], pos[2], 1.0f);
        L.P(0, i) = make_float4(h.x, h.y, h.z, h.w);
        float u = 0.0f, v = 0.0f;
        if (masked && p.texcoords) { u = p.texcoords[(size_t)vi * 2]; v = p.texcoords[(size_t)vi * 2 + 1]; }
        L.U(0, i) = u; L.V(0, i) = v;
    }
    int np = 3;
    cur = 0;
    for (int pl = p.depthClamp ? 2 : 0; pl < 6 && np >= 3; pl++) {
        int m2 = 0;
        for (int i = 0; i < np; i++) {
            const int j = (i + 1) % np;
            const float4 Pv = L.P(cur, i), Qv = L.P(cur, j);
            const f4 P = {Pv.x, Pv.y, Pv.z, Pv.w}, Q = {Qv.x, Qv.y, Qv.z, Qv.w};
            const float pui = L.U(cur, i), pvi = L.V(cur, i), puj = L.U(cur, j), pvj = L.V(cur, j);
            const float dp = clip_dist(P, pl), dq = clip_dist(Q, pl);
            const bool pin = dp >= 0.0f, qin = dq >= 0.0f;
            if (pin && m2 < CLIP_MAXV) { L.U(cur ^ 1, m2) = pui; L.V(cur ^ 1, m2) = pvi; L.P(cur ^ 1, m2) = Pv; m2++; }
            if (pin && !qin && m2 < CLIP_MAXV) {
                const float t = dp / (dp - dq);
                L.U(cur ^ 1, m2) = pui + (puj - pui) * t; L.V(cur ^ 1, m2) = pvi + (pvj - pvi) * t;
                const f4 x = clip_intersect(P, Q, dp, dq);
                L.P(cur ^ 1, m2) = make_float4(x.x, x.y, x.z, x.w); m2++;
            } else if (!pin && qin && m2 < CLIP_MAXV) {
                const float t = dq / (dq - dp);
                L.U(cur ^ 1, m2) = puj + (pui - puj) * t; L.V(cur ^ 1, m2) = pvj + (pvi - pvj) * t;
                const f4 x = clip_intersect(Q, P, dq, dp);
                L.P(cur ^ 1, m2) = make_float4(x.x, x.y, x.z, x.w); m2++;
            }
        }
        np = m2; cur ^= 1;
    }
    if (np < 3) return 0;
    for (int i = 0; i < np; i++) {
        const float4 h = L.P(cur, i);
        if (!(h.w > 0.0f)) return 0;
        const float u = h.x / fabsf(h.w) * 0.5f + 0.5f;
        const float v = h.y / fabsf(h.w) * -0.5f + 0.5f;
        L.X(i) = (int32_t)rintf((u * p.W) * 256.0f);
        L.Y(i) = (int32_t)rintf((v * p.H) * 256.0f);
        L.D(i) = h.z / h.w;
    }
    return np;
}

__device__ void raster_clip_part(const RasterParams& p, uint32_t block, uint32_t blocks)
{
    __shared__ float4 sPoly[2 * CLIP_MAXV * CLIP_THREADS];
    __shared__ float sPU[2 * CLIP_MAXV * CLIP_THREADS], sPV[2 * CLIP_MAXV * CLIP_THREADS];
    __shared__ int32_t sPX[CLIP_MAXV * CLIP_THREADS], sPY[CLIP_MAXV * CLIP_THREADS];
    __shared__ float sPD[CLIP_MAXV * CLIP_THREADS];
    if (threadIdx.x >= CLIP_THREADS) return;
    const ClipLds<CLIP_THREADS> L = {sPoly, sPU, sPV, sPX, sPY, sPD, threadIdx.x};
    const uint32_t n = min(p.counters->clipTriCount[p.pass], p.clipTriCap);
    const uint32_t listShard = block % CHORD_LIST_SHARDS;
    for (uint32_t k = block * CLIP_THREADS + threadIdx.x; k < n; k += blocks * CLIP_THREADS) {
        const ClipTri ct = p.clipTris[k];
        ChordDrawCmd cmd; cmd.objectId = ct.objectId; cmd.meshletId = ct.meshletId; cmd.slot = ct.slot;
        const DMeshlet& m = p.meshlets[cmd.meshletId];
        const uint32_t V = m.vertexTriangleCount & 0xFFu;
        const uint32_t matFlags = p.objStatic[cmd.objectId].matFlags;
        const bool twoSided = (matFlags & CHORD_MATFLAG_TWO_SIDED) != 0u || p.depthOnly != 0u;
        const bool masked = CHORD_MATFLAG_ALPHA(matFlags) == CHORD_ALPHA_MASK;
        const float* mv = p.objFrame[cmd.objectId].mvp;
        Mat4 mvp;
        for (int r = 0; r < 4; r++) for (int cc = 0; cc < 4; cc++) mvp.r[r][cc] = mv[r * 4 + cc];
        int cur;
        const int np = clip_triangle(p, L, m, V, ct.tri, mvp, masked, cur);
        if (np < 3) continue;
        const uint32_t payload = p.depthOnly ? 0u : encode_triangle_instance(ct.tri, cmd.slot);
        const uint32_t slots = masked ? 1u + CHORD_MASK_EXT_SLOTS : 1u;
        for (int i = 1; i + 1 < np; i++) {
            TriSetup ts;
            ts.X[0] = L.X(0); ts.X[1] = L.X(i); ts.X[2] = L.X(i + 1);
            ts.Y[0] = L.Y(0); ts.Y[1] = L.Y(i); ts.Y[2] = L.Y(i + 1);
            float d[3] = {L.D(0), L.D(i), L.D(i + 1)};
            ts.payload = payload;
            if (!tri_setup(ts, twoSided, p.Wi, p.Hi) || !owns_rect(p.shard, ts.px0, ts.py0, ts.px1, ts.py1)) continue;
            if (p.biasConst != 0.0f || p.biasSlope != 0.0f) { const float o = depth_bias(ts, d, p.biasConst, p.biasSlope); d[0] += o; d[1] += o; d[2] += o; }
            const uint32_t li = atomicAdd(&p.counters->triCount[listShard * CHORD_SHARD_STRIDE], slots);
            if (li + slots > p.triCap) { atomicOr(&p.counters->overflow, 1u); continue; }
            const uint32_t gi = listShard * p.triCap + li;
            write_record(&p.tris[gi], ts, d, twoSided, masked);
            if (masked) {
                const uint32_t material = CHORD_MATFLAG_MATERIAL(matFlags);
                const float u3[3] = {L.U(cur, 0), L.U(cur, i), L.U(cur, i + 1)}, v3[3] = {L.V(cur, 0), L.V(cur, i), L.V(cur, i + 1)};
                const float w3[3] = {L.P(cur, 0).w, L.P(cur, i).w, L.P(cur, i + 1).w};
                write_mask_ext(&p.tris[gi + 1u], &p.materials[material], material, ts.area, u3, v3, w3);
            }
            bin_record_tiles(p, ts, gi | (masked ? CHORD_REC_MASKED : CHORD_REC_WIDE));
        }
    }
}

#define CLIP_BLOCKS 64u
__device__ void raster_bin_large_part(const RasterParams& p, uint32_t block, uint32_t blocks)
{
    const uint32_t lane = threadIdx.x & 63u, wave = threadIdx.x >> 6;
    __shared__ uint32_t sStart[CHORD_LIST_SHARDS + 1];
    if (threadIdx.x < 64u) {
        const uint32_t cnt = min(p.counters->largeCount[p.pass][threadIdx.x * CHORD_SHARD_STRIDE], p.largeCap);
        uint32_t incl = cnt;
#pragma unroll
        for (int d = 1; d < 64; d <<= 1) { const uint32_t nb = (uint32_t)__shfl_up((int)incl, d, 64); if (lane >= (uint32_t)d) incl += nb; }
        sStart[threadIdx.x + 1u] = incl;
        if (threadIdx.x == 0u) sStart[0] = 0u;
    }
    __syncthreads();
    const uint32_t n = sStart[CHORD_LIST_SHARDS];
    for (uint32_t k = block * 4u + wave; k < n; k += blocks * 4u) {
        uint32_t sh = 0;
#pragma unroll
        for (uint32_t st = 32u; st > 0u; st >>= 1) if (sStart[sh + st] <= k) sh += st;
        const uint32_t gi = __builtin_amdgcn_readfirstlane(p.largeList[(size_t)sh * p.largeCap + (k - sStart[sh])]);
        const TriRec* __restrict__ r = &p.tris[gi];
        TriSetup ts;
#pragma unroll
        for (int i = 0; i < 3; i++) { ts.X[i] = r->X[i]; ts.Y[i] = r->Y[i]; }
        ts.payload = 0;
        if (!tri_setup(ts, (r->twoSided & 1u) != 0, p.Wi, p.Hi)) continue;
        const bool maskedRec = (r->twoSided & 4u) != 0u;
        const int ea[3] = {1, 2, 0}, eb[3] = {2, 0, 1};
        int64_t a[3], b[3], bias[3], dxe[3], dye[3];
#pragma unroll
        for (int i = 0; i < 3; i++) {
            dxe[i] = (int64_t)(ts.X[eb[i]] - ts.X[ea[i]]); dye[i] = (int64_t)(ts.Y[eb[i]] - ts.Y[ea[i]]);
            a[i] = -(int64_t)ts.s * dye[i]; b[i] = (int64_t)ts.s * dxe[i];
            bias[i] = (a[i] > 0 || (a[i] == 0 && b[i] > 0)) ? 0 : -1;
        }
        const int32_t tx0 = ts.px0 >> TILE_SHIFT, tx1 = ts.px1 >> TILE_SHIFT;
        const int32_t ty0 = ts.py0 >> TILE_SHIFT, ty1 = ts.py1 >> TILE_SHIFT;
        const uint32_t tw = (uint32_t)(tx1 - tx0 + 1), nt = tw * (uint32_t)(ty1 - ty0 + 1);
        for (uint32_t tb = 0; tb < nt; tb += 64u) {
            const uint32_t t = tb + lane;
            if (t >= nt) continue;
            const int32_t tx = tx0 + (int32_t)(t % tw), ty = ty0 + (int32_t)(t / tw);
            const int32_t rx0 = max(ts.px0, tx << TILE_SHIFT), rx1 = min(ts.px1, (tx << TILE_SHIFT) + TILE - 1);
            const int32_t ry0 = max(ts.py0, ty << TILE_SHIFT), ry1 = min(ts.py1, (ty << TILE_SHIFT) + TILE - 1);
            bool hit = owns_tile(p.shard, tx, ty);
#pragma unroll
            for (int i = 0; i < 3; i++) {
                const int64_t cx = (int64_t)(a[i] > 0 ? rx1 : rx0) * 256 + 128, cy = (int64_t)(b[i] > 0 ? ry1 : ry0) * 256 + 128;
                const int64_t E = (int64_t)ts.s * (dxe[i] * (cy - ts.Y[ea[i]]) - dye[i] * (cx - ts.X[ea[i]]));
                hit = hit && !(E + bias[i] < 0);
            }
            if (hit) {
                const uint32_t tile = (uint32_t)ty * p.tilesX + (uint32_t)tx;
                const uint32_t slot = atomicAdd(&p.tileCount[(size_t)tile * TC_STRIDE], 1u);
                bin_store(p, tile, slot, gi | (maskedRec ? CHORD_REC_MASKED : CHORD_REC_WIDE));
                if (maskedRec) p.tileCount[(size_t)tile * TC_STRIDE + TC_MASKED] = 1u;
            }
        }
    }
}

__global__ __launch_bounds__(256) void raster_clip_and_bin_large_kernel(RasterParams p)
{
    if (blockIdx.x < CLIP_BLOCKS) raster_clip_part(p, blockIdx.x, CLIP_BLOCKS);
    else raster_bin_large_part(p, blockIdx.x - CLIP_BLOCKS, gridDim.x - CLIP_BLOCKS);
}

#define TILE_SLICE_SHIFT CHORD_TILE_SLICE_SHIFT
#define TILE_SLICE (1u << TILE_SLICE_SHIFT)
#ifndef TILE_SPLIT_MIN
#define TILE_SPLIT_MIN 6144u
#endif
#ifndef TILE_ORDER_KEEP
#define TILE_ORDER_KEEP 1
#endif
#ifndef TILE_MAKE_NEXT
#define TILE_MAKE_NEXT 1
#endif
#ifndef TILE_DIRECT
#define TILE_DIRECT 1
#endif
#ifndef TILE_DIRECT_MAX_CLUSTERS
#define TILE_DIRECT_MAX_CLUSTERS 1024u
#endif
#ifndef TILE_SLICE_MIN
#define TILE_SLICE_MIN 1024u
#endif
template <uint32_t NT>
__device__ __forceinline__ void tile_order_part(const RasterParams& p, uint2* __restrict__ order)
{
    __shared__ uint32_t hist[20], base[20], cursor[20], splitItems, splitCursor, longest, hotCount, hotList[CHORD_HOT_TILES], entriesAll, tilesBusy;
    const uint32_t tiles = p.tilesX * p.tilesY;
    if (threadIdx.x < 20u) { hist[threadIdx.x] = 0; cursor[threadIdx.x] = 0; }
    if (threadIdx.x == 0) { splitItems = 0; splitCursor = 0; longest = 0; hotCount = 0; entriesAll = 0; tilesBusy = 0; }
    __syncthreads();
    auto tile_word = [&](uint32_t t) -> uint32_t {
        if (!owns_tile(p.shard, (int32_t)(t % p.tilesX), (int32_t)(t / p.tilesX))) return 0xFFFFFFFFu;
        const uint32_t* __restrict__ line = &p.tileCount[(size_t)t * TC_STRIDE];
        const uint32_t n = line[0], nb = line[1], nm = line[3];
        return min(n, bin_capacity(p)) | (nb ? 0x80000000u : 0u) | (nm ? 0x40000000u : 0u);
    };
    constexpr uint32_t PER_THREAD = CHORD_MAX_TILES / NT;
    uint32_t mine[PER_THREAD];
#pragma unroll
    for (uint32_t k = 0; k < PER_THREAD; k++) { const uint32_t t = threadIdx.x + k * NT; mine[k] = t < tiles ? tile_word(t) : 0xFFFFFFFFu; }
    uint32_t sumMine = 0, tilesMine = 0;
    if (p.tileSlots) {
#pragma unroll
        for (uint32_t k = 0; k < PER_THREAD; k++) {
            const uint32_t w = mine[k];
            if (w != 0xFFFFFFFFu) { const uint32_t c = w & 0x3FFFFFFFu; sumMine += c; tilesMine += c ? 1u : 0u; }
        }
        wave_sum2(sumMine, tilesMine);
        if ((threadIdx.x & 63u) == 0u) { atomicAdd(&entriesAll, sumMine); atomicAdd(&tilesBusy, tilesMine); }
        __syncthreads();
    }
    uint32_t splitMin = p.tileSplitMin, sliceLen = p.tileSliceLen;
    if (p.tileSlots && tilesBusy < p.tileSlots) {
        const uint32_t share = (entriesAll / p.tileSlots + 511u) & ~511u;
        sliceLen = min(p.tileSliceLen, max(TILE_SLICE_MIN, share));
        splitMin = min(p.tileSplitMin, sliceLen + sliceLen / 2u);
    }
    auto slices_of = [&](uint32_t c) -> uint32_t { return (c > splitMin && !ABL(p, DBG_NO_SPLIT)) ? min((c + sliceLen - 1u) / sliceLen, CHORD_TILE_MAX_SLICES) : 0u; };
#pragma unroll
    for (uint32_t k = 0; k < PER_THREAD; k++) {
        const uint32_t t = threadIdx.x + k * NT, w = mine[k];
        if (w == 0xFFFFFFFFu) continue;
        const uint32_t c = w & 0x3FFFFFFFu;
        if (c >= p.slotHot && p.hotTiles) { const uint32_t h = atomicAdd(&hotCount, 1u); if (h < CHORD_HOT_TILES) hotList[h] = t | (c >= SLOT_VERY_HOT ? 0x80000000u : 0u); }
        const uint32_t sl = slices_of(c);
        if (sl) {
            atomicAdd(&splitItems, sl);
            if (c > TILE_SPLIT_MIN) atomicMax(&longest, c);
        } else atomicAdd(&hist[c ? 16u - (31u - (uint32_t)__clz(c)) : 17u], 1u);
    }
    __syncthreads();
    if (threadIdx.x == 0) {
        uint32_t acc = splitItems;
        for (int b = 0; b < 18; b++) { base[b] = acc; acc += hist[b]; }
        order[0] = make_uint2((p.clearTiles || p.orderAll) ? acc : acc - hist[17], 0u);
        if (p.binHint) *p.binHint = longest;
        if (p.heavyHint) p.heavyHint[(splitItems != 0u || *p.count > TILE_DIRECT_MAX_CLUSTERS) ? 0 : 2] = p.binStamp;
        if (p.countHint) *p.countHint = *p.count;
        if (p.hotTiles) p.hotTiles[0] = min(hotCount, (uint32_t)CHORD_HOT_TILES);
    }
    if (p.hotTiles && threadIdx.x < min(hotCount, (uint32_t)CHORD_HOT_TILES)) p.hotTiles[1u + threadIdx.x] = hotList[threadIdx.x];
    __syncthreads();
#pragma unroll
    for (uint32_t k = 0; k < PER_THREAD; k++) {
        const uint32_t t = threadIdx.x + k * NT, w = mine[k];
        if (w == 0xFFFFFFFFu) continue;
        const uint32_t c = w & 0x3FFFFFFFu, sl = slices_of(c);
        if (sl) {
            const uint32_t pos = atomicAdd(&splitCursor, sl);
            for (uint32_t j = 0; j < sl; j++) order[1u + pos + j] = make_uint2(t | (j << 12) | ((sl - 1u) << 22), w);
        } else {
            const uint32_t b = c ? 16u - (31u - (uint32_t)__clz(c)) : 17u;
            order[1u + base[b] + atomicAdd(&cursor[b], 1u)] = make_uint2(t, w);
        }
    }
}

__device__ __noinline__ void tile_order_next_part(const RasterParams* q)
{
    tile_order_part<512u>(*q, q->tileOrderNext);
}

__global__ __launch_bounds__(1024) void raster_tile_order_kernel(RasterParams p)
{
    tile_order_part<1024u>(p, p.tileOrder);
}



struct WideEdges {
    int64_t a[3], b[3], bias[3], dx[3], dy[3];
    int32_t Xa[3], Ya[3];
    int32_t s;
};

__device__ __forceinline__ void wide_edges(const TriSetup& ts, WideEdges& w)
{
    const int ea[3] = {1, 2, 0}, eb[3] = {2, 0, 1};
    w.s = ts.s;
#pragma unroll
    for (int i = 0; i < 3; i++) {
        w.dx[i] = (int64_t)(ts.X[eb[i]] - ts.X[ea[i]]);
        w.dy[i] = (int64_t)(ts.Y[eb[i]] - ts.Y[ea[i]]);
        w.Xa[i] = ts.X[ea[i]]; w.Ya[i] = ts.Y[ea[i]];
        w.a[i] = -(int64_t)ts.s * w.dy[i];
        w.b[i] = (int64_t)ts.s * w.dx[i];
        w.bias[i] = (w.a[i] > 0 || (w.a[i] == 0 && w.b[i] > 0)) ? 0 : -1;
    }
}

__device__ __forceinline__ int64_t edge_at(const WideEdges& w, int i, int32_t px, int32_t py)
{
    const int64_t cx = (int64_t)px * 256 + 128, cy = (int64_t)py * 256 + 128;
    return (int64_t)w.s * (w.dx[i] * (cy - w.Ya[i]) - w.dy[i] * (cx - w.Xa[i]));
}

__device__ __forceinline__ void lds_write(unsigned long long* tile, int32_t lx, int32_t ly, float z, uint32_t payload)
{
    const unsigned long long packed = ((unsigned long long)__float_as_uint(z) << 32) | (unsigned long long)payload;
    atomicMax(&tile[ly * TPITCH + lx], packed);
}

template <int PITCH>
__device__ __forceinline__ void tile_raster_narrow(unsigned long long* tile, const TriSetup& ts, int32_t ox, int32_t oy,
                                                   int32_t x0, int32_t y0, int32_t x1, int32_t y1, bool noPixels, const bool clampZ)
{
    const bool neg = ts.s < 0;
    const int32_t dx0 = ts.X[2] - ts.X[1], dy0 = ts.Y[2] - ts.Y[1];
    const int32_t dx1 = ts.X[0] - ts.X[2], dy1 = ts.Y[0] - ts.Y[2];
    const int32_t dx2 = ts.X[1] - ts.X[0], dy2 = ts.Y[1] - ts.Y[0];
    const int32_t a0 = neg ? dy0 : -dy0, b0 = neg ? -dx0 : dx0;
    const int32_t a1 = neg ? dy1 : -dy1, b1 = neg ? -dx1 : dx1;
    const int32_t a2 = neg ? dy2 : -dy2, b2 = neg ? -dx2 : dx2;
    const int32_t bias0 = (a0 > 0 || (a0 == 0 && b0 > 0)) ? 0 : -1;
    const int32_t bias1 = (a1 > 0 || (a1 == 0 && b1 > 0)) ? 0 : -1;
    const int32_t bias2 = (a2 > 0 || (a2 == 0 && b2 > 0)) ? 0 : -1;
    const int32_t cx0 = x0 * 256 + 128, cy0 = y0 * 256 + 128;
    int32_t r0 = __mul24(b0, cy0 - ts.Y[1]) + __mul24(a0, cx0 - ts.X[1]) + bias0;
    int32_t r1 = __mul24(b1, cy0 - ts.Y[2]) + __mul24(a1, cx0 - ts.X[2]) + bias1;
    int32_t r2 = __mul24(b2, cy0 - ts.Y[0]) + __mul24(a2, cx0 - ts.X[0]) + bias2;
    int32_t E0 = r0, E1 = r1, E2 = r2;
    const int32_t w = x1 - x0 + 1, count = __mul24(w, y1 - y0 + 1);
    const int32_t sx0 = a0 * 256, sx1 = a1 * 256, sx2 = a2 * 256;
    const int32_t sw0 = b0 * 256 - __mul24(w - 1, sx0), sw1 = b1 * 256 - __mul24(w - 1, sx1), sw2 = b2 * 256 - __mul24(w - 1, sx2);
    int32_t col = 0;
    unsigned long long* px = tile + (y0 - oy) * PITCH + (x0 - ox);
    const unsigned long long payload = (unsigned long long)ts.payload;
    for (int32_t i = 0; i < count; i++) {
        const bool inside = (E0 | E1 | E2) >= 0 && !noPixels;
        const float l1 = (float)(E1 - bias1) * ts.invA, l2 = (float)(E2 - bias2) * ts.invA;
        float z = (ts.d0 + l1 * ts.e1) + l2 * ts.e2;
        if (clampZ) z = fminf(fmaxf(z, 0.0f), 1.0f);
        atomicMax(px, inside ? (((unsigned long long)__float_as_uint(z) << 32) | payload) : 0ull);
        col++;
        const bool wrap = col == w;
        E0 += wrap ? sw0 : sx0; E1 += wrap ? sw1 : sx1; E2 += wrap ? sw2 : sx2;
        px += wrap ? PITCH - w + 1 : 1;
        col = wrap ? 0 : col;
    }
}

#ifndef TINY_AREA
#define TINY_AREA 8
#endif
#ifndef TINY_AREA_DENSE
#define TINY_AREA_DENSE 48
#endif
#ifndef TINY_DENSE_MIN
#define TINY_DENSE_MIN 1024u
#endif

struct UnitParams {
    int32_t X[3], Y[3];
    float d0, e1, e2, invA;
    uint32_t payload;
    uint32_t box;
    int32_t skind;
};
#define TB 512
static_assert(TB == 512, "tile_order_part rounds a pass's slice length to batches of 512");
#define UNIT_CAP 4096

template <typename E_t>
__device__ __forceinline__ void scan_row(unsigned long long* __restrict__ tileRow, const UnitParams& u, int32_t ox, int32_t py,
                                         int32_t lx0, int32_t lx1, bool noPixels, const bool clampZ)
{
    const E_t s = (u.skind & 1) ? (E_t)-1 : (E_t)1;
    const E_t dx0 = (E_t)(u.X[2] - u.X[1]), dy0 = (E_t)(u.Y[2] - u.Y[1]);
    const E_t dx1 = (E_t)(u.X[0] - u.X[2]), dy1 = (E_t)(u.Y[0] - u.Y[2]);
    const E_t dx2 = (E_t)(u.X[1] - u.X[0]), dy2 = (E_t)(u.Y[1] - u.Y[0]);
    const E_t a0 = -s * dy0, b0 = s * dx0, a1 = -s * dy1, b1 = s * dx1, a2 = -s * dy2, b2 = s * dx2;
    const E_t bias0 = (a0 > 0 || (a0 == 0 && b0 > 0)) ? (E_t)0 : (E_t)-1;
    const E_t bias1 = (a1 > 0 || (a1 == 0 && b1 > 0)) ? (E_t)0 : (E_t)-1;
    const E_t bias2 = (a2 > 0 || (a2 == 0 && b2 > 0)) ? (E_t)0 : (E_t)-1;
    const E_t cx = (E_t)(ox + lx0) * (E_t)256 + (E_t)128, cy = (E_t)py * (E_t)256 + (E_t)128;
    E_t E0 = s * (dx0 * (cy - (E_t)u.Y[1]) - dy0 * (cx - (E_t)u.X[1])) + bias0;
    E_t E1 = s * (dx1 * (cy - (E_t)u.Y[2]) - dy1 * (cx - (E_t)u.X[2])) + bias1;
    E_t E2 = s * (dx2 * (cy - (E_t)u.Y[0]) - dy2 * (cx - (E_t)u.X[0])) + bias2;
    const E_t st0 = a0 * (E_t)256, st1 = a1 * (E_t)256, st2 = a2 * (E_t)256;
    float klo = 0.0f, khi = (float)(lx1 - lx0);
    {
        const float e[3] = {(float)E0, (float)E1, (float)E2}, t[3] = {(float)st0, (float)st1, (float)st2};
#pragma unroll
        for (int i = 0; i < 3; i++) {
            const float q = fminf(fmaxf(-e[i] * __builtin_amdgcn_rcpf(t[i]), -4.0f), 4096.0f);
            if (t[i] > 0.0f) klo = fmaxf(klo, floorf(q) - 1.0f);
            else if (t[i] < 0.0f) khi = fminf(khi, floorf(q) + 1.0f);
            else if (e[i] < 0.0f) khi = -1.0f;
        }
    }
    const int32_t k0 = (int32_t)klo, k1 = (int32_t)khi;
    E0 += (E_t)k0 * st0; E1 += (E_t)k0 * st1; E2 += (E_t)k0 * st2;
    unsigned long long* px = tileRow + lx0 + k0;
    const unsigned long long payload = noPixels ? 0ull : (unsigned long long)u.payload;
    for (int32_t k = k0; k <= k1; k++) {
        const bool inside = std::is_floating_point<E_t>::value ? (E0 >= (E_t)0 && E1 >= (E_t)0 && E2 >= (E_t)0)
                                                              : (((int64_t)E0 | (int64_t)E1 | (int64_t)E2) >= 0);
        const float l1 = (float)(double)(E1 - bias1) * u.invA, l2 = (float)(double)(E2 - bias2) * u.invA;
        float z = (u.d0 + l1 * u.e1) + l2 * u.e2;
        if (clampZ) z = fminf(fmaxf(z, 0.0f), 1.0f);
        const unsigned long long packed = ((unsigned long long)__float_as_uint(z) << 32) | payload;
        atomicMax(px, inside && !noPixels ? packed : 0ull);
        E0 += st0; E1 += st1; E2 += st2; px++;
    }
}

__device__ __forceinline__ uint32_t block_scan_tb(uint32_t v, uint32_t* waveSums, uint32_t* total)
{
    const uint32_t lane = threadIdx.x & 63u, wave = threadIdx.x >> 6;
    uint32_t incl = v;
#pragma unroll
    for (int d = 1; d < 64; d <<= 1) {
        const uint32_t nb = __shfl_up(incl, d, 64);
        if (lane >= (uint32_t)d) incl += nb;
    }
    if (lane == 63u) waveSums[wave] = incl;
    __syncthreads();
    uint32_t base = 0, tot = 0;
#pragma unroll
    for (uint32_t w = 0; w < TB / 64u; w++) { const uint32_t sw = waveSums[w]; if (w < wave) base += sw; tot += sw; }
    *total = tot;
    return base + incl - v;
}


#ifndef SEG_SHIFT
#define SEG_SHIFT 6
#endif
#define SEG (1 << SEG_SHIFT)
#ifndef MASKED_ROWS
#define MASKED_ROWS 1
#endif
#ifndef MASKED_SEG_SHIFT
#define MASKED_SEG_SHIFT 6
#endif
#define MASKED_SEG (1 << MASKED_SEG_SHIFT)
#ifndef MASKED_PIXELS_PER_TRIP
#define MASKED_PIXELS_PER_TRIP 1
#endif
#define ENTRY_WORDS 13
#ifndef TILE_BATCH
#define TILE_BATCH TB
#endif
#ifndef TILE_UNIT_CAP
#define TILE_UNIT_CAP UNIT_CAP
#endif
struct EntrySoA { uint32_t w[ENTRY_WORDS][TILE_BATCH]; };
#define EF_KIND_SHIFT 24

template <typename E_t>
__device__ __forceinline__ int32_t scan_span(unsigned long long* __restrict__ tileRow, E_t E0, E_t E1, E_t E2, E_t st0, E_t st1, E_t st2,
                                          E_t bias1, E_t bias2, float d0, float e1, float e2, float invA, uint32_t payloadIn,
                                          int32_t lx0, int32_t lx1, bool noPixels, const bool clampZ = false)
{
    float klo = 0.0f, khi = (float)(lx1 - lx0);
    {
// ... 718 lines not shown
                uint32_t seg = nseg == 1u ? 0u : nseg == 2u ? (j & 1u) : nseg == 4u ? (j & 3u) : j % 3u;
                for (uint32_t u = lo2; u < hi2; u++) {
                    unitList[u - r0] = tix | (row << 9) | (seg << 15);
                    if (++seg == nseg) { seg = 0u; row++; }
                }
            }
        };
        for (uint32_t r0 = 0; r0 < total; r0 += TILE_UNIT_CAP) {
            list_units(offN, rowsN, r0);
            __syncthreads();
            const uint32_t nr = min(total - r0, (uint32_t)TILE_UNIT_CAP);
            for (uint32_t ui = tix; ui < nr; ui += TB) {
                const uint32_t d = unitList[ui];
                if (ABL(p, DBG_NO_UNITS)) continue;
                const int32_t trips = entry_unit<MASKED, DEPTH>(p, prm, tile, d & 511u, (d >> 9) & 63u, (d >> 15) & 3u, ox, oy, noPixels);
                if (prof) { cUnits++; cUnitIters += (uint32_t)trips; }
            }
            if (r0 + TILE_UNIT_CAP < total || totalM) __syncthreads();
        }
        for (uint32_t r0 = 0; r0 < totalM; r0 += TILE_UNIT_CAP) {
            if (rowsM) {
                const uint32_t box = prm.w[11][tix];
                const uint32_t nseg = ((((box >> 12) & 63u) - (box & 63u)) >> MASKED_SEG_SHIFT) + 1u, y0l = (box >> 6) & 63u;
                const uint32_t lo2 = max(offM, r0), hi2 = min(offM + rowsM, r0 + TILE_UNIT_CAP);
                if (lo2 < hi2) {
                    const uint32_t j = lo2 - offM, g = j / nseg;
                    uint32_t row = y0l + g * MASKED_ROWS, seg = j - g * nseg;
                    for (uint32_t u = lo2; u < hi2; u++) {
                        unitList[u - r0] = tix | (row << 9) | (seg << 15);
                        if (++seg == nseg) { seg = 0u; row += MASKED_ROWS; }
                    }
                }
            }
            __syncthreads();
            const uint32_t nr = min(totalM - r0, (uint32_t)TILE_UNIT_CAP);
            for (uint32_t ui = tix; ui < nr; ui += TB) {
                const uint32_t d = unitList[ui];
                entry_unit_masked<DEPTH>(p, prm, tile, d & 511u, (d >> 9) & 63u, (d >> 15) & 7u, ox, oy, noPixels);
            }
            if (r0 + TILE_UNIT_CAP < totalM) __syncthreads();
        }
        total |= totalM;
        if (total) __syncthreads();
        PHASE(4);
    };
    uint32_t batchNo = 0;
    if constexpr (TILE_DEEP_FETCH && !MASKED) {
        uint32_t nameA = nameNext, nameB = idxNext;
        uint4 b0 = make_uint4(0, 0, 0, 0), b1 = b0, b2 = b0;
        if (nameB != 0xFFFFFFFFu) FETCH_REC(nameB, b0, b1, b2);
        uint32_t idx = entryThread && k0 + 2u * TILE_BATCH < n ? binEntry(k0 + 2u * TILE_BATCH) : 0xFFFFFFFFu;
        for (uint32_t base = lo; base < n;) {
            window_advance(base);
            uint32_t rows = batch_setup(nq0, nq1, nq2, nameA);
            nameA = idx;
            if (nameA != 0xFFFFFFFFu) FETCH_REC(nameA, nq0, nq1, nq2);
            idx = entryThread && base + tix + 3u * TILE_BATCH < n ? binEntry(base + tix + 3u * TILE_BATCH) : 0xFFFFFFFFu;
            batch_units(rows, batchNo);
            base += TILE_BATCH; batchNo++;
            if (base >= n) break;
            window_advance(base);
            rows = batch_setup(b0, b1, b2, nameB);
            nameB = idx;
            if (nameB != 0xFFFFFFFFu) FETCH_REC(nameB, b0, b1, b2);
            idx = entryThread && base + tix + 3u * TILE_BATCH < n ? binEntry(base + tix + 3u * TILE_BATCH) : 0xFFFFFFFFu;
            batch_units(rows, batchNo);
            base += TILE_BATCH; batchNo++;
        }
    } else
    for (uint32_t base = lo; base < n; base += TILE_BATCH, batchNo++) {
        window_advance(base);
        const uint32_t k = base + tix;
        const uint4 q0 = nq0, q1 = nq1, q2 = nq2;
        const uint32_t name = nameNext;
        nameNext = idxNext;
        if (nameNext != 0xFFFFFFFFu) FETCH_REC(nameNext, nq0, nq1, nq2);
        idxNext = entryThread && k + 2u * TILE_BATCH < n ? binEntry(k + 2u * TILE_BATCH) : 0xFFFFFFFFu;
        batch_units(batch_setup(q0, q1, q2, name), batchNo);
    }
    __syncthreads();

    if (mergeSlices) {
        const RasterParams* q = kernel_args();
        if (!merge_slices(tile, scalar_load(&q->tileSlabs) + (size_t)tileId * (TILE * TILE), &scalar_load(&q->tileCount)[(size_t)tileId * TC_STRIDE + TC_TICKET],
                          slices, &sTicket, &scalar_load(&q->counters)->overflow)) continue;
        if (rmw) {
            for (uint32_t i = tix, visBase = vis_base(); i < TILE * TILE / 2; i += TB) {
                const int32_t ly = (int32_t)(i >> (TILE_SHIFT - 1)), lx = (int32_t)(i & (TILE / 2 - 1)) * 2;
                if (ly >= th || lx >= tw) continue;
                const unsigned long long* src = p.vis + (size_t)(visBase + (uint32_t)ly * visPitch + (uint32_t)lx);
                tile[ly * TPITCH + lx] = max(tile[ly * TPITCH + lx], src[0]);
                if (lx + 1 < tw) tile[ly * TPITCH + lx + 1] = max(tile[ly * TPITCH + lx + 1], src[1]);
            }
        }
        __syncthreads();
    }

    if (ABL(p, DBG_NO_OUT)) {
    } else if (p.hzbFused && !ABL(p, DBG_NO_HZB)) {
        tile_out_and_hzb<SH>(tile, reinterpret_cast<float*>(&prm.w[0][0]), offs, tileId, slot_of_tile(), nAll, ox, oy, tw, th);
    } else if (p.clearTiles || p.hzbFused) {
        for (uint32_t i = tix, visBase = vis_base(); i < TILE * TILE / 2; i += TB) {
            const int32_t ly = (int32_t)(i >> (TILE_SHIFT - 1)), lx = (int32_t)(i & (TILE / 2 - 1)) * 2;
            if (ly >= th || lx >= tw) continue;
            const ulonglong2 v = make_ulonglong2(tile[ly * TPITCH + lx], tile[ly * TPITCH + lx + 1]);
            unsigned long long* dst = p.vis + (size_t)(visBase + (uint32_t)ly * visPitch + (uint32_t)lx);
            if (lx + 1 < tw) *reinterpret_cast<ulonglong2*>(dst) = v;
            else dst[0] = v.x;
        }
    } else {
        for (uint32_t i = tix, visBase = vis_base(); i < TILE * TILE; i += TB) {
            const int32_t ly = (int32_t)(i >> TILE_SHIFT), lx = (int32_t)(i & (TILE - 1));
            const unsigned long long v = tile[ly * TPITCH + lx];
            if (v != 0ull && ly < th && lx < tw) atomicMax(p.vis + (size_t)(visBase + (uint32_t)ly * visPitch + (uint32_t)lx), v);
        }
    }
    PHASE(5);
    if (prof) {
        if (tix == 0) {
            p.tileClocks[tileId] = wall_clock64() - t0;
            for (int i = 0; i < 6; i++) p.tilePhase[(size_t)tileId * 8 + i] = ph[i];
            p.tilePhase[(size_t)tileId * 8 + 6] = 0ull; p.tilePhase[(size_t)tileId * 8 + 7] = 0ull;
        }
        __syncthreads();
        atomicAdd(&p.tilePhase[(size_t)tileId * 8 + 6], ((unsigned long long)cUnits << 32) | cUnitIters);
        atomicAdd(&p.tilePhase[(size_t)tileId * 8 + 7], ((unsigned long long)cTiny << 32) | cTinyIters);
        if ((tix & 63u) == 0u) for (int i = 0; i < 6; i++) atomicAdd(&p.tilePhase[(size_t)tileId * 8 + i], bw[i] << 32);
    }
    __syncthreads();
    }
}
#undef wgs
#undef TILE_SKEW

#if !CHORD_MASKED_FUSED && TILE_BATCH != TB
#error "the separate masked pass sets up one entry per thread of its workgroup: TILE_BATCH must be TB"
#endif
#if TILE_BATCH == TB
template <bool SH, bool DEPTH>
__global__ __launch_bounds__(TB, 4) void raster_masked_tile_kernel(RasterParams p)
{
    __shared__ __align__(16) unsigned long long tile[TILE * TPITCH];
    __shared__ EntrySoA prm;
    __shared__ uint32_t unitList[UNIT_CAP];
    __shared__ uint32_t waveSums[2][TB / 64];
    __shared__ uint32_t chunkTab[64];
    const uint32_t active = p.tileOrder[0].x;
    for (uint32_t oi = blockIdx.x; oi < active; oi += gridDim.x) {
    const uint2 item = p.tileOrder[1u + oi];
    if ((item.y & 0x40000000u) == 0u || ((item.x >> 12) & 0x3FFu) != 0u) continue;
    const uint32_t tileId = item.x & 0xFFFu;
    const uint32_t n = item.y & 0x3FFFFFFFu;
    const int32_t ox = (int32_t)(tileId % p.tilesX) * TILE, oy = (int32_t)(tileId / p.tilesX) * TILE;
    const int32_t tw = min(TILE, p.Wi - ox), th = min(TILE, p.Hi - oy);
    const bool noPixels = ABL(p, DBG_NO_PIXELS);
    for (uint32_t i = threadIdx.x; i < TILE * TPITCH / 2; i += TB) reinterpret_cast<ulonglong2*>(tile)[i] = make_ulonglong2(0ull, 0ull);
    const uint32_t* bin = p.tileBins + (size_t)tileId * p.binCap;
    const uint32_t wideLimit = min(p.triCap * CHORD_LIST_SHARDS, CHORD_REC_WIDE_INDEX);
    uint32_t batch = 0;
    for (uint32_t segLo = 0; segLo < n;) {
        uint32_t segHi, chunk0 = 0;
        if (segLo < p.binCap) segHi = min(n, p.binCap);
        else {
            chunk0 = (segLo - p.binCap) >> CHORD_BIN_CHUNK_SHIFT;
            segHi = min(n, segLo + 64u * CHORD_BIN_CHUNK);
            __syncthreads();
            for (uint32_t j = threadIdx.x; j < 64u; j += TB) {
                const unsigned long long e = chunk0 + j < p.binMaxChunks ? p.binChunkTab[(size_t)tileId * p.binMaxChunks + chunk0 + j] : 0ull;
                chunkTab[j] = (uint32_t)(e >> 32) == p.binStamp ? (uint32_t)e : CHORD_BIN_CHUNK_INVALID;
            }
        }
        __syncthreads();
        auto binWord = [&](uint32_t k) -> uint32_t {
            if (k < p.binCap) return bin[k];
            const uint32_t o = k - p.binCap, cj = (o >> CHORD_BIN_CHUNK_SHIFT) - chunk0;
            const uint32_t id = cj < 64u ? chunkTab[cj] : CHORD_BIN_CHUNK_INVALID;
            return id == CHORD_BIN_CHUNK_INVALID ? 0xFFFFFFFFu : p.binPool[(size_t)id * CHORD_BIN_CHUNK + (o & (CHORD_BIN_CHUNK - 1u))];
        };
        uint32_t wNext = segLo + threadIdx.x < segHi ? binWord(segLo + threadIdx.x) : 0xFFFFFFFFu;
        for (uint32_t base = segLo; base < segHi; base += TB, batch++) {
            const uint32_t w = wNext;
            wNext = base + TB + threadIdx.x < segHi ? binWord(base + TB + threadIdx.x) : 0xFFFFFFFFu;
            const uint32_t idx = w & CHORD_REC_WIDE_INDEX;
            uint32_t units = 0;
            if ((w & 0xE0000000u) == CHORD_REC_MASKED && idx < wideLimit) {
                const uint4* src = reinterpret_cast<const uint4*>(&p.tris[idx]);
                const uint4 q0 = src[0], q1 = src[1], q2 = src[2];
                TriRec r;
                r.X[0] = (int32_t)q0.x; r.X[1] = (int32_t)q0.y; r.X[2] = (int32_t)q0.z; r.Y[0] = (int32_t)q0.w;
                r.Y[1] = (int32_t)q1.x; r.Y[2] = (int32_t)q1.y;
                r.d[0] = __uint_as_float(q1.z); r.d[1] = __uint_as_float(q1.w); r.d[2] = __uint_as_float(q2.x);
                r.payload = q2.y; r.twoSided = q2.z; r.pad = q2.w;
                TriSetup ts;
                tri_setup_from_record(ts, r, p.Wi, p.Hi);
                const int32_t x0 = max(ts.px0, ox), y0 = max(ts.py0, oy);
                const int32_t x1 = min(ts.px1, ox + tw - 1), y1 = min(ts.py1, oy + th - 1);
                if (x1 >= x0 && y1 >= y0) units = entry_store(prm, threadIdx.x, ts, narrow_extent(ts), ox, oy, x0, y0, x1, y1, true, idx);
            }
            uint32_t total;
            const uint32_t off = block_scan_tb(units, waveSums[batch & 1u], &total);
            for (uint32_t r0 = 0; r0 < total; r0 += UNIT_CAP) {
                if (units) {
                    const uint32_t box = prm.w[11][threadIdx.x];
                    const uint32_t nseg = ((((box >> 12) & 63u) - (box & 63u)) >> MASKED_SEG_SHIFT) + 1u, y0l = (box >> 6) & 63u;
                    const uint32_t lo2 = max(off, r0), hi2 = min(off + units, r0 + UNIT_CAP);
                    if (lo2 < hi2) {
                        const uint32_t j = lo2 - off, g = j / nseg;
                        uint32_t row = y0l + g * MASKED_ROWS, seg = j - g * nseg;
                        for (uint32_t u = lo2; u < hi2; u++) {
                            unitList[u - r0] = threadIdx.x | (row << 9) | (seg << 15);
                            if (++seg == nseg) { seg = 0u; row += MASKED_ROWS; }
                        }
                    }
                }
                __syncthreads();
                const uint32_t nr = min(total - r0, (uint32_t)UNIT_CAP);
                for (uint32_t ui = threadIdx.x; ui < nr; ui += TB) {
                    const uint32_t d = unitList[ui];
                    entry_unit_masked<DEPTH>(p, prm, tile, d & 511u, (d >> 9) & 63u, (d >> 15) & 7u, ox, oy, noPixels);
                }
                if (r0 + UNIT_CAP < total) __syncthreads();
            }
            if (total) __syncthreads();
        }
        segLo = segHi;
    }
    __syncthreads();
    const uint32_t visBase = SH ? p.shard.tileSlot[tileId] << (2 * TILE_SHIFT) : (uint32_t)oy * (uint32_t)p.Wi + (uint32_t)ox;
    const uint32_t visPitch = SH ? (uint32_t)TILE : (uint32_t)p.Wi;
    if (p.clearTiles) {
        for (uint32_t i = threadIdx.x; i < TILE * TILE / 2; i += TB) {
            const int32_t ly = (int32_t)(i >> (TILE_SHIFT - 1)), lx = (int32_t)(i & (TILE / 2 - 1)) * 2;
            if (ly >= th || lx >= tw) continue;
            const ulonglong2 v = make_ulonglong2(tile[ly * TPITCH + lx], tile[ly * TPITCH + lx + 1]);
            unsigned long long* dst = p.vis + (size_t)(visBase + (uint32_t)ly * visPitch + (uint32_t)lx);
            if (lx + 1 < tw) *reinterpret_cast<ulonglong2*>(dst) = v;
            else dst[0] = v.x;
        }
    } else {
        for (uint32_t i = threadIdx.x; i < TILE * TILE; i += TB) {
            const int32_t ly = (int32_t)(i >> TILE_SHIFT), lx = (int32_t)(i & (TILE - 1));
            const unsigned long long v = tile[ly * TPITCH + lx];
            if (v != 0ull && ly < th && lx < tw) atomicMax(p.vis + (size_t)(visBase + (uint32_t)ly * visPitch + (uint32_t)lx), v);
        }
    }
    __syncthreads();
    }
}
#endif

hipError_t launch_raster(ChordCtx* c, const CmdList& in, bool clearTiles)
{
#define LR_HIP(call) do { const hipError_t e_ = (call); if (e_ != hipSuccess) return e_; } while (0)
    RasterParams p;
    p.hzbFused = 0; p.hzbMinA = nullptr; p.hzbMinB = nullptr; p.hzbMaxB = nullptr; p.tileRange = c->dTileRange;
    p.hzbExA = nullptr; p.hzbExB = nullptr;
    p.hzbDesc = c->hzb[0].desc;
    if (c->fuseHzb && c->shard.ranks == 1) {
        p.hzbFused = 1;
        p.hzbMinA = (clearTiles && c->fuseHzbTemp) ? c->hzb[0].minTexels : nullptr;
        p.hzbMinB = c->hzb[c->fuseHzbSlot].minTexels; p.hzbMaxB = c->hzb[c->fuseHzbSlot].maxTexels;
    } else if (c->fuseHzb) {
        p.hzbFused = 1;
        p.hzbExA = (clearTiles && c->fuseHzbTemp) ? c->dHzbExchange : nullptr;
        p.hzbExB = c->dHzbFinalExchange;
    }
    p.count = in.count; p.cmds = in.cmds; p.cmdCap = std::max(in.capacity, 1u);
    if (c->shard.ranks > 1) {
        bool mine = false;
        if (in.cmds == c->lists[0].cmds && c->mineValid) { p.count = c->dCounts + 4; p.cmds = c->dMineCmds; mine = true; }
        else if (in.cmds == c->dMineCmds && c->mineValid) mine = true;
        else for (int k = 1; k < 3; k++) if (in.cmds == c->lists[k].cmds && c->listMine[k]) mine = true;
        if (!mine) {
            if (!c->dRankCmds) LR_HIP(hipMalloc((void**)&c->dRankCmds, sizeof(ChordDrawCmd) * (size_t)c->cmdCapacity));
            CmdList filtered;
            filtered.count = c->dCounts + 5; filtered.cmds = c->dRankCmds; filtered.capacity = in.capacity;
            LR_HIP(hipMemsetAsync(filtered.count, 0, sizeof(uint32_t), c->stream));
            launch_rank_filter(c, in, filtered);
            p.count = filtered.count; p.cmds = filtered.cmds;
        }
    }
    p.objFrame = c->dObjFrame; p.objStatic = c->dObjStatic;
    p.meshlets = c->dMeshlets; p.meshletData = c->dMeshletData; p.positions = c->dPositions;
    p.materials = c->dMaterials; p.texAlpha = c->dTexAlpha; p.texcoords = c->dTexcoords;
    p.vis = (unsigned long long*)c->dVis;
    p.depthOut = (p.hzbFused && clearTiles) ? c->depthOutTarget : nullptr;
    p.W = (float)c->width; p.H = (float)c->height; p.Wi = (int32_t)c->width; p.Hi = (int32_t)c->height;
    p.shard = c->shard;
    p.blockPool = c->dBlockPool; p.blockCap = (c->debugFlags & DBG_NO_BLOCKS) ? 0u : c->blockCap;
    p.blockForce = (c->debugFlags & DBG_FORCE_BLOCKS) ? 1u : 0u;
    p.tris = c->dTris; p.triCap = c->triCap / CHORD_LIST_SHARDS;
    p.trisC = c->dTrisC; p.triCapC = c->triCapC / CHORD_LIST_SHARDS;
    const uint32_t tiles = c->tilesX * c->tilesY;
    const uint32_t pass = c->rasterCalls & 1u;
    p.tileCount = c->dFrameState->tileCount + (size_t)pass * tiles * TC_STRIDE;
    p.tileBins = c->dTileBins + (size_t)pass * tiles * c->binCap; p.binCap = c->binCap;
    p.binPool = c->dBinPool + (size_t)pass * c->binPoolChunks * CHORD_BIN_CHUNK; p.binPoolChunks = c->binPoolChunks;
    p.binPoolCount = &c->dCounters->binPoolCount[pass];
    p.binChunkTab = c->dBinChunkTab + (size_t)pass * tiles * c->binMaxChunks; p.binMaxChunks = c->binMaxChunks;
    p.binStamp = ++c->rasterSerial;
    p.tilesX = c->tilesX; p.tilesY = c->tilesY;
    p.clipTris = c->dClipTris + (size_t)pass * (c->clipTriCap / 2); p.clipTriCap = c->clipTriCap / 2; p.pass = pass;
    p.largeList = c->dLargeList + (size_t)pass * (c->largeCap / 2); p.largeCap = c->largeCap / 2 / CHORD_LIST_SHARDS;
    p.counters = c->dCounters;
    p.clearTiles = clearTiles ? 1u : 0u;
    p.depthOnly = c->depthOnly ? 1u : 0u; p.depthClamp = c->depthClamp ? 1u : 0u;
    p.biasConst = c->depthBiasConst; p.biasSlope = c->depthBiasSlope;
    p.debug = c->debugFlags;
    p.tileClocks = c->dTileClocks + (size_t)pass * CHORD_MAX_TILES;
    p.tileOrder = reinterpret_cast<uint2*>(c->dTileOrder); p.tileSlabs = c->dTileSlabs;
    p.tilePhase = c->dTileClocks + (size_t)2 * CHORD_MAX_TILES + (size_t)pass * CHORD_MAX_TILES * 8;

    if (!c->inFrame || c->rasterCalls >= 2) {
        LR_HIP(hipMemsetAsync(p.tileCount, 0, sizeof(uint32_t) * TC_STRIDE * tiles, c->stream));
        LR_HIP(hipMemsetAsync(&c->dCounters->clipTriCount[pass], 0, sizeof(uint32_t), c->stream));
        LR_HIP(hipMemsetAsync(c->dCounters->largeCount[pass], 0, sizeof(c->dCounters->largeCount[pass]), c->stream));
        LR_HIP(hipMemsetAsync(&c->dCounters->binPoolCount[pass], 0, sizeof(uint32_t), c->stream));
        if (!c->inFrame) { LR_HIP(hipMemsetAsync(c->dCounters->triCount, 0, sizeof(c->dCounters->triCount), c->stream));
                           LR_HIP(hipMemsetAsync(c->dCounters->triCountC, 0, sizeof(c->dCounters->triCountC), c->stream));
                           LR_HIP(hipMemsetAsync(c->dCounters->blockGranules, 0, sizeof(c->dCounters->blockGranules), c->stream)); }
    }

    const uint64_t rankPixels = (uint64_t)c->width * c->height / (c->shard.ranks > 1 ? c->shard.ranks : 1u);
    const bool maybeDense = p.blockCap != 0u && (p.blockForce != 0u || (uint64_t)in.capacity * 16ull >= rankPixels);
    p.leftCount = nullptr; p.leftCmds = nullptr;
    p.binHint = nullptr; p.countHint = nullptr;
    p.slotHot = (c->debugFlags & DBG_FORCE_HOT) ? 64u : SLOT_HOT;
    {
        static const int forced = [] { const char* e = getenv("CHORDVIS_TILE_SLOTS"); return e ? atoi(e) : -1; }();
        p.tileSlots = forced >= 0 ? (uint32_t)forced : c->shard.ranks > 1 ? (uint32_t)c->numCUs * (CHORD_TILE_SHIFT == 6 ? 2u : 6u) : 0u;
        static const int splitMin = [] { const char* e = getenv("CHORDVIS_TILE_SPLIT_MIN"); return e ? atoi(e) : -1; }();
        static const int sliceLen = [] { const char* e = getenv("CHORDVIS_TILE_SLICE"); return e ? atoi(e) : -1; }();
        p.tileSplitMin = splitMin > 0 ? (uint32_t)splitMin : TILE_SPLIT_MIN;
        p.tileSliceLen = sliceLen >= 512 ? ((uint32_t)sliceLen + 511u) & ~511u : TILE_SLICE;
    }
    p.hotTiles = c->dHotTiles ? c->dHotTiles + (size_t)pass * (1u + CHORD_HOT_TILES) : nullptr;
    bool blocksWorthLaunching = maybeDense;
    if (maybeDense && c->dBinHint) {
        p.countHint = c->dBinHint + 2 + pass;
        const uint32_t last = c->hBinHint[2 + pass];
        if (p.blockForce == 0u && last != 0xFFFFFFFFu && (uint64_t)last * 32ull < rankPixels) blocksWorthLaunching = false;
    }
    if (blocksWorthLaunching) {
        if (c->dBinHint) p.binHint = c->dBinHint + pass;
        if (!c->dLeftCmds) LR_HIP(hipMalloc((void**)&c->dLeftCmds, sizeof(ChordDrawCmd) * (size_t)c->cmdCapacity));
        p.leftCount = c->dCounts + 6 + pass; p.leftCmds = c->dLeftCmds;
        if (!c->inFrame || c->rasterCalls >= 2) LR_HIP(hipMemsetAsync(p.leftCount, 0, sizeof(uint32_t), c->stream));
    }
    uint32_t blocks = (in.capacity + 3u) / 4u;
#ifndef SETUP_GRID_MULT
#define SETUP_GRID_MULT 1u
#endif
    const uint32_t maxBlocks = (uint32_t)c->numCUs * SETUP_MIN_WAVES * SETUP_GRID_MULT;
    if (blocks > maxBlocks) blocks = maxBlocks;
    if (blocks < 1) blocks = 1;
    const bool sh = c->shard.ranks > 1;
    stamp(c, S_HZBCULL);
    if (blocksWorthLaunching) {
        const uint32_t bb = std::max(1u, std::min((in.capacity + 3u) / 4u, (uint32_t)c->numCUs * BLOCKS_MIN_WAVES));
        const bool hot = (c->hBinHint && c->hBinHint[pass] >= SLOT_HOT) || (c->debugFlags & DBG_FORCE_HOT);
        if (hot) CHORD_LAUNCH(c, raster_setup_blocks_kernel<true>, dim3(bb), dim3(256), 0, c->stream, p);
        else     CHORD_LAUNCH(c, raster_setup_blocks_kernel<false>, dim3(bb), dim3(256), 0, c->stream, p);
    }
    if (c->anyMasked) CHORD_LAUNCH(c, raster_setup_kernel<true>, dim3(blocks), dim3(256), 0, c->stream, p);
    else              CHORD_LAUNCH(c, raster_setup_kernel<false>, dim3(blocks), dim3(256), 0, c->stream, p);
    stamp(c, S_R_CLUSTER);
    CHORD_LAUNCH(c, raster_clip_and_bin_large_kernel, dim3(CLIP_BLOCKS + (uint32_t)c->numCUs * 4u), dim3(256), 0, c->stream, p);
    p.orderKept = 0u;
    p.heavyHint = nullptr;
    bool makeOrder = true;
    static const bool directOn = [] { const char* e = getenv("CHORDVIS_TILE_DIRECT"); return !e || atoi(e) != 0; }();
    const bool laterOk = c->inFrame && !clearTiles && p.hzbFused && !c->depthOnly && CHORD_MASKED_FUSED && c->dBinHint && !(c->debugFlags & ~(DBG_NO_BLOCKS | DBG_FORCE_BLOCKS | DBG_FORCE_HOT | 524288u));
    if (laterOk) p.heavyHint = c->dBinHint + 4 + pass;
    if (TILE_DIRECT && directOn && laterOk) {
        const uint32_t heavySeen = c->hBinHint[4 + pass], lightSeen = c->hBinHint[6 + pass];
        if (lightSeen != 0u && (heavySeen == 0u || (int32_t)(lightSeen - heavySeen) > 0)) {
            p.orderKept = 2u; makeOrder = false;
        }
    }
    p.orderAll = 0u; p.tileOrderNext = nullptr;
    static const bool keepLaterOn = [] { const char* e = getenv("CHORDVIS_TILE_KEEP_LATER"); return !e || atoi(e) != 0; }();
    static const bool nextOn = [] { const char* e = getenv("CHORDVIS_TILE_NEXT"); return !e || atoi(e) != 0; }();
    const bool keepOk = TILE_ORDER_KEEP && c->orderKeepFrames && CHORD_MASKED_FUSED && c->inFrame && !c->depthOnly && !(c->debugFlags & ~524288u);
    int slot = -1;
    if (keepOk && clearTiles && pass == 0u && c->dTileOrderKeep) slot = 0;
    else if (keepOk && keepLaterOn && laterOk && pass == 1u && c->dTileOrderKeep1) slot = 1;
    if (slot >= 0) {
        uint32_t& age = slot ? c->orderAge1 : c->orderAge;
        uint2* buf = reinterpret_cast<uint2*>(slot ? c->dTileOrderKeep1 : c->dTileOrderKeep);
        const size_t half = (size_t)1 + c->tileItemCap;
        p.orderAll = slot ? 1u : 0u;
        if (nextOn && p.orderKept == 2u) {
            age = 0xFFFFFFFFu; p.orderAll = 0u;
        } else if (nextOn) {
            uint32_t& flip = c->orderFlip[slot];
            p.tileOrder = buf + flip * half; p.tileOrderNext = buf + (flip ^ 1u) * half;
            if (age != 0xFFFFFFFFu) { p.orderKept = 1u; makeOrder = false; }
            age = 0u; flip ^= 1u;
        } else if (p.orderKept != 2u) {
            p.tileOrder = buf;
            if (age < c->orderKeepFrames) { age++; p.orderKept = 1u; makeOrder = false; }
            else age = 0u;
        } else p.orderAll = 0u;
    }
    if (makeOrder) CHORD_LAUNCH(c, raster_tile_order_kernel, dim3(1), dim3(1024), 0, c->stream, p);
#if !CHORD_MASKED_FUSED
    if (c->anyMasked) {
        const uint32_t items = tiles;
        if (c->depthClamp && !sh) CHORD_LAUNCH(c, (raster_masked_tile_kernel<false, true>), dim3(items), dim3(TB), 0, c->stream, p);
        else if (sh)              CHORD_LAUNCH(c, (raster_masked_tile_kernel<true, false>), dim3(items), dim3(TB), 0, c->stream, p);
        else                      CHORD_LAUNCH(c, (raster_masked_tile_kernel<false, false>), dim3(items), dim3(TB), 0, c->stream, p);
    }
#endif
    stamp(c, S_R_CLIP);
    const uint32_t tileBlocks = (p.tileOrderNext ? 1u : 0u) + ((clearTiles || p.orderKept == 2u || p.orderAll) ? ((sh && clearTiles) ? min(tiles, max(c->shard.slotsPerRank, p.tileSlots + p.tileSlots / 2u)) : tiles) : min(tiles, (uint32_t)c->numCUs * (CHORD_TILE_SHIFT == 6 ? 2u : 6u)));
#if CHORD_MASKED_FUSED
    if (c->anyMasked) {
        if (c->depthClamp && !sh) CHORD_LAUNCH(c, (raster_tile_kernel<false, true, true>), dim3(tileBlocks), dim3(TB), 0, c->stream, p);
        else if (sh)              CHORD_LAUNCH(c, (raster_tile_kernel<true, true, false>), dim3(tileBlocks), dim3(TB), 0, c->stream, p);
        else                      CHORD_LAUNCH(c, (raster_tile_kernel<false, true, false>), dim3(tileBlocks), dim3(TB), 0, c->stream, p);
    } else
#endif
    if (c->depthClamp && !sh) {
        CHORD_LAUNCH(c, (raster_tile_kernel<false, false, true>), dim3(tileBlocks), dim3(TB), 0, c->stream, p);
    } else {
        if (sh) CHORD_LAUNCH(c, (raster_tile_kernel<true, false, false>), dim3(tileBlocks), dim3(TB), 0, c->stream, p);
        else    CHORD_LAUNCH(c, (raster_tile_kernel<false, false, false>), dim3(tileBlocks), dim3(TB), 0, c->stream, p);
    }
    stamp(c, S_R_CHUNK);
    c->rasterCalls++;
    return hipSuccess;
#undef LR_HIP
}

}
```

Before: 3.231 Gtri/s.

## Fuse clipping and large-triangle binning into setup kernel for later passes

Moves near-plane/guard-band clipping and large-triangle tile binning out of the separate clip_and_bin_large kernel and into the setup kernel, using a per-wave chain of clip batches stored in the large list and the wave's LDS region. The separate kernel launch is skipped when enabled, which by default is pass 1 and later. The aim is to remove a launch and the global round trip of large and clip lists. In exchange the setup waves become more divergent and heavier, with clipping done on 8 lanes per wave, and the LDS layout of the setup kernel is reshaped.

After: 3.243 Gtri/s (median of 6 runs). Within noise of the previous version (+0.4%).

```diff
diff --git a/chord_amd/csrc/kernels_raster.hip b/chord_amd/csrc/kernels_raster.hip
--- a/chord_amd/csrc/kernels_raster.hip
+++ b/chord_amd/csrc/kernels_raster.hip
@@ -43,6 +43,7 @@
     uint32_t blockForce;
     ClipTri* clipTris; uint32_t clipTriCap; uint32_t pass;
     uint32_t* largeList; uint32_t largeCap;
+    uint32_t setupBins;
     DeviceCounters* counters;
     uint2* tileOrder;
     unsigned long long* tileSlabs;
@@ -319,7 +320,8 @@
     if (id != CHORD_BIN_CHUNK_INVALID) p.binPool[((size_t)id << CHORD_BIN_CHUNK_SHIFT) + (o & (CHORD_BIN_CHUNK - 1u))] = gi;
 }
 
-__device__ __forceinline__ void bin_store(const RasterParams& p, uint32_t tile, uint32_t slot, uint32_t gi)
+template <class P>
+__device__ __forceinline__ void bin_store(const P& p, uint32_t tile, uint32_t slot, uint32_t gi)
 {
     bin_alloc(p, tile, slot);
     bin_put(p, tile, slot, gi);
@@ -594,6 +596,238 @@
     a = (uint32_t)__builtin_amdgcn_readlane((int)a, 63); b = (uint32_t)__builtin_amdgcn_readlane((int)b, 63);
 }
 
+__device__ void bin_record_tiles(const RasterParams& p, const TriSetup& ts, uint32_t gi)
+{
+    const int ea[3] = {1, 2, 0}, eb[3] = {2, 0, 1};
+    const int32_t tx0 = ts.px0 >> TILE_SHIFT, tx1 = ts.px1 >> TILE_SHIFT;
+    const int32_t ty0 = ts.py0 >> TILE_SHIFT, ty1 = ts.py1 >> TILE_SHIFT;
+    for (int32_t ty = ty0; ty <= ty1; ty++)
+        for (int32_t tx = tx0; tx <= tx1; tx++) {
+            const int32_t rx0 = max(ts.px0, tx << TILE_SHIFT), rx1 = min(ts.px1, (tx << TILE_SHIFT) + TILE - 1);
+            const int32_t ry0 = max(ts.py0, ty << TILE_SHIFT), ry1 = min(ts.py1, (ty << TILE_SHIFT) + TILE - 1);
+            bool hit = owns_tile(p.shard, tx, ty);
+#pragma unroll
+            for (int i = 0; i < 3; i++) {
+                const int64_t dxe = (int64_t)(ts.X[eb[i]] - ts.X[ea[i]]), dye = (int64_t)(ts.Y[eb[i]] - ts.Y[ea[i]]);
+                const int64_t a = -(int64_t)ts.s * dye, b = (int64_t)ts.s * dxe;
+                const int64_t bias = (a > 0 || (a == 0 && b > 0)) ? 0 : -1;
+                const int64_t cx = (int64_t)(a > 0 ? rx1 : rx0) * 256 + 128, cy = (int64_t)(b > 0 ? ry1 : ry0) * 256 + 128;
+                hit = hit && !((int64_t)ts.s * (dxe * (cy - ts.Y[ea[i]]) - dye * (cx - ts.X[ea[i]])) + bias < 0);
+            }
+            if (!hit) continue;
+            const uint32_t tile = (uint32_t)ty * p.tilesX + (uint32_t)tx;
+            const uint32_t slot = atomicAdd(&p.tileCount[(size_t)tile * TC_STRIDE], 1u);
+            bin_store(p, tile, slot, gi);
+            if ((gi & 0xE0000000u) == CHORD_REC_MASKED) p.tileCount[(size_t)tile * TC_STRIDE + TC_MASKED] = 1u;
+        }
+}
+
+__device__ __forceinline__ float clip_dist(const f4& v, int k)
+{
+    switch (k) {
+    case 0: return v.w - v.z;
+    case 1: return v.z;
+    case 2: return GUARD_BAND * v.w + v.x;
+    case 3: return GUARD_BAND * v.w - v.x;
+    case 4: return GUARD_BAND * v.w + v.y;
+    default: return GUARD_BAND * v.w - v.y;
+    }
+}
+
+__device__ __forceinline__ f4 clip_intersect(const f4& in, const f4& out, float din, float dout)
+{
+    const float t = din / (din - dout);
+    f4 r;
+    r.x = in.x + (out.x - in.x) * t;
+    r.y = in.y + (out.y - in.y) * t;
+    r.z = in.z + (out.z - in.z) * t;
+    r.w = in.w + (out.w - in.w) * t;
+    return r;
+}
+
+#define CLIP_MAXV 10
+#define CLIP_THREADS 64u
+template <uint32_t STRIDE>
+struct ClipLds {
+    float4* poly; float* pu; float* pv; int32_t* px; int32_t* py; float* pd; uint32_t tl;
+    __device__ __forceinline__ float4& P(int bf, int i) const { return poly[((uint32_t)bf * CLIP_MAXV + (uint32_t)i) * STRIDE + tl]; }
+    __device__ __forceinline__ float& U(int bf, int i) const { return pu[((uint32_t)bf * CLIP_MAXV + (uint32_t)i) * STRIDE + tl]; }
+    __device__ __forceinline__ float& V(int bf, int i) const { return pv[((uint32_t)bf * CLIP_MAXV + (uint32_t)i) * STRIDE + tl]; }
+    __device__ __forceinline__ int32_t& X(int i) const { return px[(uint32_t)i * STRIDE + tl]; }
+    __device__ __forceinline__ int32_t& Y(int i) const { return py[(uint32_t)i * STRIDE + tl]; }
+    __device__ __forceinline__ float& D(int i) const { return pd[(uint32_t)i * STRIDE + tl]; }
+};
+
+template <uint32_t STRIDE>
+__device__ __forceinline__ int clip_triangle(const RasterParams& p, const ClipLds<STRIDE>& L, const DMeshlet& m, uint32_t V, uint32_t tri,
+                                             const Mat4& mvp, bool masked, int& cur)
+{
+    const uint32_t packedIdx = p.meshletData[m.dataOffset + V + tri];
+    for (int i = 0; i < 3; i++) {
+        const uint32_t li = (packedIdx >> (8 * i)) & 0xFFu;
+        const uint32_t vi = p.meshletData[m.dataOffset + li] + m.vertexBase;
+        const float* pos = p.positions + (size_t)vi * 3;
+        const f4 h = mul_mv(mvp, pos[0], pos[1], pos[2], 1.0f);
+        L.P(0, i) = make_float4(h.x, h.y, h.z, h.w);
+        float u = 0.0f, v = 0.0f;
+        if (masked && p.texcoords) { u = p.texcoords[(size_t)vi * 2]; v = p.texcoords[(size_t)vi * 2 + 1]; }
+        L.U(0, i) = u; L.V(0, i) = v;
+    }
+    int np = 3;
+    cur = 0;
+    for (int pl = p.depthClamp ? 2 : 0; pl < 6 && np >= 3; pl++) {
+        int m2 = 0;
+        for (int i = 0; i < np; i++) {
+            const int j = (i + 1) % np;
+            const float4 Pv = L.P(cur, i), Qv = L.P(cur, j);
+            const f4 P = {Pv.x, Pv.y, Pv.z, Pv.w}, Q = {Qv.x, Qv.y, Qv.z, Qv.w};
+            const float pui = L.U(cur, i), pvi = L.V(cur, i), puj = L.U(cur, j), pvj = L.V(cur, j);
+            const float dp = clip_dist(P, pl), dq = clip_dist(Q, pl);
+            const bool pin = dp >= 0.0f, qin = dq >= 0.0f;
+            if (pin && m2 < CLIP_MAXV) { L.U(cur ^ 1, m2) = pui; L.V(cur ^ 1, m2) = pvi; L.P(cur ^ 1, m2) = Pv; m2++; }
+            if (pin && !qin && m2 < CLIP_MAXV) {
+                const float t = dp / (dp - dq);
+                L.U(cur ^ 1, m2) = pui + (puj - pui) * t; L.V(cur ^ 1, m2) = pvi + (pvj - pvi) * t;
+                const f4 x = clip_intersect(P, Q, dp, dq);
+                L.P(cur ^ 1, m2) = make_float4(x.x, x.y, x.z, x.w); m2++;
+            } else if (!pin && qin && m2 < CLIP_MAXV) {
+                const float t = dq / (dq - dp);
+                L.U(cur ^ 1, m2) = puj + (pui - puj) * t; L.V(cur ^ 1, m2) = pvj + (pvi - pvj) * t;
+                const f4 x = clip_intersect(Q, P, dq, dp);
+                L.P(cur ^ 1, m2) = make_float4(x.x, x.y, x.z, x.w); m2++;
+            }
+        }
+        np = m2; cur ^= 1;
+    }
+    if (np < 3) return 0;
+    for (int i = 0; i < np; i++) {
+        const float4 h = L.P(cur, i);
+        if (!(h.w > 0.0f)) return 0;
+        const float u = h.x / fabsf(h.w) * 0.5f + 0.5f;
+        const float v = h.y / fabsf(h.w) * -0.5f + 0.5f;
+        L.X(i) = (int32_t)rintf((u * p.W) * 256.0f);
+        L.Y(i) = (int32_t)rintf((v * p.H) * 256.0f);
+        L.D(i) = h.z / h.w;
+    }
+    return np;
+}
+
+template <uint32_t STRIDE>
+__device__ __forceinline__ void clip_emit(const RasterParams& p, const ClipLds<STRIDE>& L, const ClipTri& ct, uint32_t listShard)
+{
+    ChordDrawCmd cmd; cmd.objectId = ct.objectId; cmd.meshletId = ct.meshletId; cmd.slot = ct.slot;
+    const DMeshlet& m = p.meshlets[cmd.meshletId];
+    const uint32_t V = m.vertexTriangleCount & 0xFFu;
+    const uint32_t matFlags = p.objStatic[cmd.objectId].matFlags;
+    const bool twoSided = (matFlags & CHORD_MATFLAG_TWO_SIDED) != 0u || p.depthOnly != 0u;
+    const bool masked = CHORD_MATFLAG_ALPHA(matFlags) == CHORD_ALPHA_MASK;
+    const float* mv = p.objFrame[cmd.objectId].mvp;
+    Mat4 mvp;
+    for (int r = 0; r < 4; r++) for (int cc = 0; cc < 4; cc++) mvp.r[r][cc] = mv[r * 4 + cc];
+    int cur;
+    const int np = clip_triangle(p, L, m, V, ct.tri, mvp, masked, cur);
+    if (np < 3) return;
+    const uint32_t payload = p.depthOnly ? 0u : encode_triangle_instance(ct.tri, cmd.slot);
+    const uint32_t slots = masked ? 1u + CHORD_MASK_EXT_SLOTS : 1u;
+    for (int i = 1; i + 1 < np; i++) {
+        TriSetup ts;
+        ts.X[0] = L.X(0); ts.X[1] = L.X(i); ts.X[2] = L.X(i + 1);
+        ts.Y[0] = L.Y(0); ts.Y[1] = L.Y(i); ts.Y[2] = L.Y(i + 1);
+        float d[3] = {L.D(0), L.D(i), L.D(i + 1)};
+        ts.payload = payload;
+        if (!tri_setup(ts, twoSided, p.Wi, p.Hi) || !owns_rect(p.shard, ts.px0, ts.py0, ts.px1, ts.py1)) continue;
+        if (p.biasConst != 0.0f || p.biasSlope != 0.0f) { const float o = depth_bias(ts, d, p.biasConst, p.biasSlope); d[0] += o; d[1] += o; d[2] += o; }
+        const uint32_t li = atomicAdd(&p.counters->triCount[listShard * CHORD_SHARD_STRIDE], slots);
+        if (li + slots > p.triCap) { atomicOr(&p.counters->overflow, 1u); continue; }
+        const uint32_t gi = listShard * p.triCap + li;
+        write_record(&p.tris[gi], ts, d, twoSided, masked);
+        if (masked) {
+            const uint32_t material = CHORD_MATFLAG_MATERIAL(matFlags);
+            const float u3[3] = {L.U(cur, 0), L.U(cur, i), L.U(cur, i + 1)}, v3[3] = {L.V(cur, 0), L.V(cur, i), L.V(cur, i + 1)};
+            const float w3[3] = {L.P(cur, 0).w, L.P(cur, i).w, L.P(cur, i + 1).w};
+            write_mask_ext(&p.tris[gi + 1u], &p.materials[material], material, ts.area, u3, v3, w3);
+        }
+        bin_record_tiles(p, ts, gi | (masked ? CHORD_REC_MASKED : CHORD_REC_WIDE));
+    }
+}
+
+template <class P>
+__device__ __forceinline__ void bin_large_record(const P& p, uint32_t gi, uint32_t lane, int32_t Wi, int32_t Hi)
+{
+    const TriRec* __restrict__ r = &p.tris[gi];
+    TriSetup ts;
+#pragma unroll
+    for (int i = 0; i < 3; i++) { ts.X[i] = r->X[i]; ts.Y[i] = r->Y[i]; }
+    ts.payload = 0;
+    if (!tri_setup(ts, (r->twoSided & 1u) != 0, Wi, Hi)) return;
+    const bool maskedRec = (r->twoSided & 4u) != 0u;
+    gi |= maskedRec ? CHORD_REC_MASKED : CHORD_REC_WIDE;
+    const int ea[3] = {1, 2, 0}, eb[3] = {2, 0, 1};
+    int64_t a[3], b[3], bias[3], dxe[3], dye[3];
+#pragma unroll
+    for (int i = 0; i < 3; i++) {
+        dxe[i] = (int64_t)(ts.X[eb[i]] - ts.X[ea[i]]); dye[i] = (int64_t)(ts.Y[eb[i]] - ts.Y[ea[i]]);
+        a[i] = -(int64_t)ts.s * dye[i]; b[i] = (int64_t)ts.s * dxe[i];
+        bias[i] = (a[i] > 0 || (a[i] == 0 && b[i] > 0)) ? 0 : -1;
+    }
+    const int32_t tx0 = ts.px0 >> TILE_SHIFT, tx1 = ts.px1 >> TILE_SHIFT;
+    const int32_t ty0 = ts.py0 >> TILE_SHIFT, ty1 = ts.py1 >> TILE_SHIFT;
+    const uint32_t tw = (uint32_t)(tx1 - tx0 + 1), nt = tw * (uint32_t)(ty1 - ty0 + 1);
+    for (uint32_t tb = 0; tb < nt; tb += 64u) {
+        const uint32_t t = tb + lane;
+        if (t >= nt) continue;
+        const int32_t tx = tx0 + (int32_t)(t % tw), ty = ty0 + (int32_t)(t / tw);
+        const int32_t rx0 = max(ts.px0, tx << TILE_SHIFT), rx1 = min(ts.px1, (tx << TILE_SHIFT) + TILE - 1);
+        const int32_t ry0 = max(ts.py0, ty << TILE_SHIFT), ry1 = min(ts.py1, (ty << TILE_SHIFT) + TILE - 1);
+        bool hit = owns_tile(p.shard, tx, ty);
+#pragma unroll
+        for (int i = 0; i < 3; i++) {
+            const int64_t cx = (int64_t)(a[i] > 0 ? rx1 : rx0) * 256 + 128, cy = (int64_t)(b[i] > 0 ? ry1 : ry0) * 256 + 128;
+            const int64_t E = (int64_t)ts.s * (dxe[i] * (cy - ts.Y[ea[i]]) - dye[i] * (cx - ts.X[ea[i]]));
+            hit = hit && !(E + bias[i] < 0);
+        }
+        if (hit) {
+            const uint32_t tile = (uint32_t)ty * p.tilesX + (uint32_t)tx;
+            const uint32_t slot = atomicAdd(&p.tileCount[(size_t)tile * TC_STRIDE], 1u);
+            bin_store(p, tile, slot, gi);
+            if (maskedRec) p.tileCount[(size_t)tile * TC_STRIDE + TC_MASKED] = 1u;
+        }
+    }
+}
+
+#define WAVE_LDS_SYNC() do { __builtin_amdgcn_fence(__ATOMIC_RELEASE, "wavefront"); __builtin_amdgcn_wave_barrier(); __builtin_amdgcn_fence(__ATOMIC_ACQUIRE, "wavefront"); } while (0)
+
+#define SETUP_CLIP_LANES 8u
+__device__ __forceinline__ void setup_clip_chain(float* region, uint32_t chain, uint32_t listShard)
+{
+    constexpr uint32_t R = SETUP_CLIP_LANES;
+    static_assert((4u + 2u + 2u) * 2u * CLIP_MAXV * R + 3u * CLIP_MAXV * R <= 6u * LDS_VERTS, "clip polygons exceed the wave's LDS region");
+    const RasterParams& p = *kernel_args();
+    const uint32_t lane = threadIdx.x & 63u;
+    float4* poly = reinterpret_cast<float4*>(region);
+    float* pu = region + 4u * 2u * CLIP_MAXV * R;
+    float* pv = pu + 2u * CLIP_MAXV * R;
+    int32_t* px = reinterpret_cast<int32_t*>(pv + 2u * CLIP_MAXV * R);
+    int32_t* py = px + CLIP_MAXV * R;
+    float* pd = reinterpret_cast<float*>(py + CLIP_MAXV * R);
+    const ClipLds<R> L = {poly, pu, pv, px, py, pd, lane};
+    __builtin_amdgcn_fence(__ATOMIC_RELEASE, "workgroup");
+    __builtin_amdgcn_wave_barrier();
+    __builtin_amdgcn_fence(__ATOMIC_ACQUIRE, "workgroup");
+    for (uint32_t r = chain, r0 = 0u; r != 0u; ) {
+        const uint32_t first = (r - 1u) >> 7, n = ((r - 1u) & 127u) + 1u;
+        if (lane < R && r0 + lane < n) {
+            ClipTri ct = p.clipTris[first + r0 + lane];
+            ct.objectId = __builtin_amdgcn_readfirstlane(ct.objectId); ct.meshletId = __builtin_amdgcn_readfirstlane(ct.meshletId);
+            ct.slot = __builtin_amdgcn_readfirstlane(ct.slot);
+            clip_emit(p, L, ct, listShard);
+        }
+        WAVE_LDS_SYNC();
+        r0 += R;
+        if (r0 >= n) { r = __builtin_amdgcn_readfirstlane(p.largeList[first]); r0 = 0u; }
+    }
+}
+
 enum { K_NONE = 0, K_EMIT = 1, K_CLIP = 2 };
 #define WIN CHORD_BLOCK_WIN
 #define DBG_NO_BLOCKS 32768u
@@ -601,12 +835,12 @@
 #define DBG_FORCE_HOT 262144u
 
 template <bool MASKED>
-__device__ __forceinline__ void raster_setup_body(const RasterParams& p, const ChordDrawCmd* __restrict__ cmds, const uint32_t count, float (*sVert)[4][LDS_VERTS],
+__device__ __forceinline__ void raster_setup_body(const RasterParams& p, const ChordDrawCmd* __restrict__ cmds, const uint32_t count, float (*sVert)[6][LDS_VERTS],
                                                   const uint32_t firstCmd0, const uint32_t firstCmd1, const uint32_t firstCmd2, const bool firstCmdValid)
 {
     const uint32_t lane = threadIdx.x & 63u, wave = threadIdx.x >> 6;
-    float* lX = sVert[0][wave]; float* lY = sVert[1][wave]; float* lW = sVert[2][wave];
-    float* lU = sVert[3][wave]; float* lV = sVert[4][wave]; float* lD = sVert[5][wave];
+    float* lX = sVert[wave][0]; float* lY = sVert[wave][1]; float* lW = sVert[wave][2];
+    float* lU = sVert[wave][3]; float* lV = sVert[wave][4]; float* lD = sVert[wave][5];
 
     const uint32_t listShard = (blockIdx.x * 4u + wave) % CHORD_LIST_SHARDS;
 
@@ -645,6 +879,11 @@
     const uint32_t stride = gridDim.x * 4u;
     uint32_t c = blockIdx.x * 4u + wave;
     if (c >= count) return;
+    const bool sprof = RASTER_PROFILE && (p.debug & DBG_SETUP_CLOCKS) != 0;
+    unsigned long long sph[5] = {0, 0, 0, 0, 0}, stp = sprof ? wall_clock64() : 0ull;
+#define SPHASE(i) do { if (sprof) { const unsigned long long tn = wall_clock64(); sph[i] += tn - stp; stp = tn; } } while (0)
+    const uint32_t laneTop = lane;
+    uint32_t clipChain = 0u;
     Header hdr = firstCmdValid ? header_of(firstCmd0, firstCmd1, firstCmd2) : load_header(c);
     Header hdrN = load_header(c + stride);
     Mat4 mvpNext = mvp_of(hdr.objectId);
@@ -661,10 +900,6 @@
         const float* __restrict__ pb = ps + (size_t)(ib * 3u);
         pax = pa[0]; pay = pa[1]; paz = pa[2]; pbx = pb[0]; pby = pb[1]; pbz = pb[2];
     }
-    const bool sprof = RASTER_PROFILE && (p.debug & DBG_SETUP_CLOCKS) != 0;
-    unsigned long long sph[5] = {0, 0, 0, 0, 0}, stp = sprof ? wall_clock64() : 0ull;
-#define SPHASE(i) do { if (sprof) { const unsigned long long tn = wall_clock64(); sph[i] += tn - stp; stp = tn; } } while (0)
-    const uint32_t laneTop = lane;
     for (; c < count; c += stride) {
         uint32_t lane = laneTop;
         asm volatile("" : "+v"(lane));
@@ -804,6 +1039,11 @@
                 if (k < e.clipTriCap) { ClipTri ct; ct.objectId = hdr.objectId; ct.meshletId = hdr.meshletId; ct.slot = hdr.slot; ct.tri = lane + 64u; e.clipTris[k] = ct; }
                 else atomicOr(&e.counters->overflow, 2u);
             }
+            const bool selfBin = scalar_load(&kernel_args()->setupBins) != 0u;
+            if (selfBin && nClip != 0u && cbase < e.clipTriCap) {
+                if (lane == 0u) e.largeList[cbase] = clipChain;
+                clipChain = ((cbase << 7) | (min(nClip, e.clipTriCap - cbase) - 1u)) + 1u;
+            }
             uint32_t giA = 0, giB = 0;
             bool okA = false, okB = false;
             if (cpA) {
@@ -831,13 +1071,23 @@
                 } else atomicOr(&e.counters->overflow, 1u);
             }
             if (emA | emB) wave_bin_commit(e, ticket, okA, giA, okB, giB);
+            bool bgA = false, bgB = false;
             if (lgA && okA) {
                 const uint32_t k = lbase + (uint32_t)__popcll(lmA & lt);
-                if (k < e.largeCap) e.largeList[(size_t)listShard * e.largeCap + k] = giA & CHORD_REC_WIDE_INDEX; else atomicOr(&e.counters->overflow, 1u);
+                if (k < e.largeCap) { if (selfBin) bgA = true; else e.largeList[(size_t)listShard * e.largeCap + k] = giA & CHORD_REC_WIDE_INDEX; }
+                else atomicOr(&e.counters->overflow, 1u);
             }
             if (lgB && okB) {
                 const uint32_t k = lbase + (uint32_t)__popcll(lmA) + (uint32_t)__popcll(lmB & lt);
-                if (k < e.largeCap) e.largeList[(size_t)listShard * e.largeCap + k] = giB & CHORD_REC_WIDE_INDEX; else atomicOr(&e.counters->overflow, 1u);
+                if (k < e.largeCap) { if (selfBin) bgB = true; else e.largeList[(size_t)listShard * e.largeCap + k] = giB & CHORD_REC_WIDE_INDEX; }
+                else atomicOr(&e.counters->overflow, 1u);
+            }
+            const unsigned long long bmA = __ballot(bgA), bmB = __ballot(bgB);
+            if ((bmA | bmB) != 0ull) {
+                __builtin_amdgcn_fence(__ATOMIC_RELEASE, "workgroup");
+                __builtin_amdgcn_fence(__ATOMIC_ACQUIRE, "workgroup");
+                for (unsigned long long m = bmA; m != 0ull; m &= m - 1ull) bin_large_record(e, bcast(giA, __builtin_ctzll(m)) & CHORD_REC_WIDE_INDEX, lane, p.Wi, p.Hi);
+                for (unsigned long long m = bmB; m != 0ull; m &= m - 1ull) bin_large_record(e, bcast(giB, __builtin_ctzll(m)) & CHORD_REC_WIDE_INDEX, lane, p.Wi, p.Hi);
             }
             }
         }
@@ -849,6 +1099,7 @@
         pax = nax; pay = nay; paz = naz; pbx = nbx; pby = nby; pbz = nbz;
         SPHASE(4);
     }
+    if (clipChain != 0u) setup_clip_chain(lX, clipChain, listShard);
     if (sprof && lane == 0u) {
         const uint32_t w = blockIdx.x * 4u + wave;
         if (w < CHORD_MAX_TILES * 8u / 5u) for (int i = 0; i < 5; i++) p.tilePhase[(size_t)w * 5u + i] = sph[i];
@@ -876,8 +1127,6 @@
     e.counters = scalar_load(&q->counters);
     return e;
 }
-
-#define WAVE_LDS_SYNC() do { __builtin_amdgcn_fence(__ATOMIC_RELEASE, "wavefront"); __builtin_amdgcn_wave_barrier(); __builtin_amdgcn_fence(__ATOMIC_ACQUIRE, "wavefront"); } while (0)
 
 __device__ __forceinline__ int classify_triangle(const RasterParams& p, uint32_t t, uint32_t T, uint32_t packedIdx, bool twoSided, bool allFast,
                                                  const float* lX, const float* lY, const float* lW, const float* lU, const float* lV, const float* lD,
@@ -1227,7 +1476,7 @@
 template <bool MASKED>
 __global__ __launch_bounds__(256, MASKED ? SETUP_MASKED_WAVES : SETUP_MIN_WAVES) void raster_setup_kernel(RasterParams p)
 {
-    __shared__ float sVert[6][4][LDS_VERTS];
+    __shared__ float sVert[4][6][LDS_VERTS];
     const uint32_t c0 = __builtin_amdgcn_readfirstlane(min(blockIdx.x * 4u + (threadIdx.x >> 6), p.cmdCap - 1u));
     const uint32_t* __restrict__ cw = reinterpret_cast<const uint32_t*>(p.cmds + c0);
     const uint32_t f0 = scalar_load(cw), f1 = scalar_load(cw + 1), f2 = scalar_load(cw + 2);
@@ -1250,122 +1499,6 @@
     raster_setup_blocks_body<HOT>(p, count, sVert, sSnap, sWin, sSlots);
 }
 
-__device__ void bin_record_tiles(const RasterParams& p, const TriSetup& ts, uint32_t gi)
-{
-    const int ea[3] = {1, 2, 0}, eb[3] = {2, 0, 1};
-    const int32_t tx0 = ts.px0 >> TILE_SHIFT, tx1 = ts.px1 >> TILE_SHIFT;
-    const int32_t ty0 = ts.py0 >> TILE_SHIFT, ty1 = ts.py1 >> TILE_SHIFT;
-    for (int32_t ty = ty0; ty <= ty1; ty++)
-        for (int32_t tx = tx0; tx <= tx1; tx++) {
-            const int32_t rx0 = max(ts.px0, tx << TILE_SHIFT), rx1 = min(ts.px1, (tx << TILE_SHIFT) + TILE - 1);
-            const int32_t ry0 = max(ts.py0, ty << TILE_SHIFT), ry1 = min(ts.py1, (ty << TILE_SHIFT) + TILE - 1);
-            bool hit = owns_tile(p.shard, tx, ty);
-#pragma unroll
-            for (int i = 0; i < 3; i++) {
-                const int64_t dxe = (int64_t)(ts.X[eb[i]] - ts.X[ea[i]]), dye = (int64_t)(ts.Y[eb[i]] - ts.Y[ea[i]]);
-                const int64_t a = -(int64_t)ts.s * dye, b = (int64_t)ts.s * dxe;
-                const int64_t bias = (a > 0 || (a == 0 && b > 0)) ? 0 : -1;
-                const int64_t cx = (int64_t)(a > 0 ? rx1 : rx0) * 256 + 128, cy = (int64_t)(b > 0 ? ry1 : ry0) * 256 + 128;
-                hit = hit && !((int64_t)ts.s * (dxe * (cy - ts.Y[ea[i]]) - dye * (cx - ts.X[ea[i]])) + bias < 0);
-            }
-            if (!hit) continue;
-            const uint32_t tile = (uint32_t)ty * p.tilesX + (uint32_t)tx;
-            const uint32_t slot = atomicAdd(&p.tileCount[(size_t)tile * TC_STRIDE], 1u);
-            bin_store(p, tile, slot, gi);
-            if ((gi & 0xE0000000u) == CHORD_REC_MASKED) p.tileCount[(size_t)tile * TC_STRIDE + TC_MASKED] = 1u;
-        }
-}
-
-__device__ __forceinline__ float clip_dist(const f4& v, int k)
-{
-    switch (k) {
-    case 0: return v.w - v.z;
-    case 1: return v.z;
-    case 2: return GUARD_BAND * v.w + v.x;
-    case 3: return GUARD_BAND * v.w - v.x;
-    case 4: return GUARD_BAND * v.w + v.y;
-    default: return GUARD_BAND * v.w - v.y;
-    }
-}
-
-__device__ __forceinline__ f4 clip_intersect(const f4& in, const f4& out, float din, float dout)
-{
-    const float t = din / (din - dout);
-    f4 r;
-    r.x = in.x + (out.x - in.x) * t;
-    r.y = in.y + (out.y - in.y) * t;
-    r.z = in.z + (out.z - in.z) * t;
-    r.w = in.w + (out.w - in.w) * t;
-    return r;
-}
-
-#define CLIP_MAXV 10
-#define CLIP_THREADS 64u
-template <uint32_t STRIDE>
-struct ClipLds {
-    float4* poly; float* pu; float* pv; int32_t* px; int32_t* py; float* pd; uint32_t tl;
-    __device__ __forceinline__ float4& P(int bf, int i) const { return poly[((uint32_t)bf * CLIP_MAXV + (uint32_t)i) * STRIDE + tl]; }
-    __device__ __forceinline__ float& U(int bf, int i) const { return pu[((uint32_t)bf * CLIP_MAXV + (uint32_t)i) * STRIDE + tl]; }
-    __device__ __forceinline__ float& V(int bf, int i) const { return pv[((uint32_t)bf * CLIP_MAXV + (uint32_t)i) * STRIDE + tl]; }
-    __device__ __forceinline__ int32_t& X(int i) const { return px[(uint32_t)i * STRIDE + tl]; }
-    __device__ __forceinline__ int32_t& Y(int i) const { return py[(uint32_t)i * STRIDE + tl]; }
-    __device__ __forceinline__ float& D(int i) const { return pd[(uint32_t)i * STRIDE + tl]; }
-};
-
-template <uint32_t STRIDE>
-__device__ __forceinline__ int clip_triangle(const RasterParams& p, const ClipLds<STRIDE>& L, const DMeshlet& m, uint32_t V, uint32_t tri,
-                                             const Mat4& mvp, bool masked, int& cur)
-{
-    const uint32_t packedIdx = p.meshletData[m.dataOffset + V + tri];
-    for (int i = 0; i < 3; i++) {
-        const uint32_t li = (packedIdx >> (8 * i)) & 0xFFu;
-        const uint32_t vi = p.meshletData[m.dataOffset + li] + m.vertexBase;
-        const float* pos = p.positions + (size_t)vi * 3;
-        const f4 h = mul_mv(mvp, pos[0], pos[1], pos[2], 1.0f);
-        L.P(0, i) = make_float4(h.x, h.y, h.z, h.w);
-        float u = 0.0f, v = 0.0f;
-        if (masked && p.texcoords) { u = p.texcoords[(size_t)vi * 2]; v = p.texcoords[(size_t)vi * 2 + 1]; }
-        L.U(0, i) = u; L.V(0, i) = v;
-    }
-    int np = 3;
-    cur = 0;
-    for (int pl = p.depthClamp ? 2 : 0; pl < 6 && np >= 3; pl++) {
-        int m2 = 0;
-        for (int i = 0; i < np; i++) {
-            const int j = (i + 1) % np;
-            const float4 Pv = L.P(cur, i), Qv = L.P(cur, j);
-            const f4 P = {Pv.x, Pv.y, Pv.z, Pv.w}, Q = {Qv.x, Qv.y, Qv.z, Qv.w};
-            const float pui = L.U(cur, i), pvi = L.V(cur, i), puj = L.U(cur, j), pvj = L.V(cur, j);
-            const float dp = clip_dist(P, pl), dq = clip_dist(Q, pl);
-            const bool pin = dp >= 0.0f, qin = dq >= 0.0f;
-            if (pin && m2 < CLIP_MAXV) { L.U(cur ^ 1, m2) = pui; L.V(cur ^ 1, m2) = pvi; L.P(cur ^ 1, m2) = Pv; m2++; }
-            if (pin && !qin && m2 < CLIP_MAXV) {
-                const float t = dp / (dp - dq);
-                L.U(cur ^ 1, m2) = pui + (puj - pui) * t; L.V(cur ^ 1, m2) = pvi + (pvj - pvi) * t;
-                const f4 x = clip_intersect(P, Q, dp, dq);
-                L.P(cur ^ 1, m2) = make_float4(x.x, x.y, x.z, x.w); m2++;
-            } else if (!pin && qin && m2 < CLIP_MAXV) {
-                const float t = dq / (dq - dp);
-                L.U(cur ^ 1, m2) = puj + (pui - puj) * t; L.V(cur ^ 1, m2) = pvj + (pvi - pvj) * t;
-                const f4 x = clip_intersect(Q, P, dq, dp);
-                L.P(cur ^ 1, m2) = make_float4(x.x, x.y, x.z, x.w); m2++;
-            }
-        }
-        np = m2; cur ^= 1;
-    }
-    if (np < 3) return 0;
-    for (int i = 0; i < np; i++) {
-        const float4 h = L.P(cur, i);
-        if (!(h.w > 0.0f)) return 0;
-        const float u = h.x / fabsf(h.w) * 0.5f + 0.5f;
-        const float v = h.y / fabsf(h.w) * -0.5f + 0.5f;
-        L.X(i) = (int32_t)rintf((u * p.W) * 256.0f);
-        L.Y(i) = (int32_t)rintf((v * p.H) * 256.0f);
-        L.D(i) = h.z / h.w;
-    }
-    return np;
-}
-
 __device__ void raster_clip_part(const RasterParams& p, uint32_t block, uint32_t blocks)
 {
     __shared__ float4 sPoly[2 * CLIP_MAXV * CLIP_THREADS];
@@ -1376,43 +1509,7 @@
     const ClipLds<CLIP_THREADS> L = {sPoly, sPU, sPV, sPX, sPY, sPD, threadIdx.x};
     const uint32_t n = min(p.counters->clipTriCount[p.pass], p.clipTriCap);
     const uint32_t listShard = block % CHORD_LIST_SHARDS;
-    for (uint32_t k = block * CLIP_THREADS + threadIdx.x; k < n; k += blocks * CLIP_THREADS) {
-        const ClipTri ct = p.clipTris[k];
-        ChordDrawCmd cmd; cmd.objectId = ct.objectId; cmd.meshletId = ct.meshletId; cmd.slot = ct.slot;
-        const DMeshlet& m = p.meshlets[cmd.meshletId];
-        const uint32_t V = m.vertexTriangleCount & 0xFFu;
-        const uint32_t matFlags = p.objStatic[cmd.objectId].matFlags;
-        const bool twoSided = (matFlags & CHORD_MATFLAG_TWO_SIDED) != 0u || p.depthOnly != 0u;
-        const bool masked = CHORD_MATFLAG_ALPHA(matFlags) == CHORD_ALPHA_MASK;
-        const float* mv = p.objFrame[cmd.objectId].mvp;
-        Mat4 mvp;
-        for (int r = 0; r < 4; r++) for (int cc = 0; cc < 4; cc++) mvp.r[r][cc] = mv[r * 4 + cc];
-        int cur;
-        const int np = clip_triangle(p, L, m, V, ct.tri, mvp, masked, cur);
-        if (np < 3) continue;
-        const uint32_t payload = p.depthOnly ? 0u : encode_triangle_instance(ct.tri, cmd.slot);
-        const uint32_t slots = masked ? 1u + CHORD_MASK_EXT_SLOTS : 1u;
-        for (int i = 1; i + 1 < np; i++) {
-            TriSetup ts;
-            ts.X[0] = L.X(0); ts.X[1] = L.X(i); ts.X[2] = L.X(i + 1);
-            ts.Y[0] = L.Y(0); ts.Y[1] = L.Y(i); ts.Y[2] = L.Y(i + 1);
-            float d[3] = {L.D(0), L.D(i), L.D(i + 1)};
-            ts.payload = payload;
-            if (!tri_setup(ts, twoSided, p.Wi, p.Hi) || !owns_rect(p.shard, ts.px0, ts.py0, ts.px1, ts.py1)) continue;
-            if (p.biasConst != 0.0f || p.biasSlope != 0.0f) { const float o = depth_bias(ts, d, p.biasConst, p.biasSlope); d[0] += o; d[1] += o; d[2] += o; }
-            const uint32_t li = atomicAdd(&p.counters->triCount[listShard * CHORD_SHARD_STRIDE], slots);
-            if (li + slots > p.triCap) { atomicOr(&p.counters->overflow, 1u); continue; }
-            const uint32_t gi = listShard * p.triCap + li;
-            write_record(&p.tris[gi], ts, d, twoSided, masked);
-            if (masked) {
-                const uint32_t material = CHORD_MATFLAG_MATERIAL(matFlags);
-                const float u3[3] = {L.U(cur, 0), L.U(cur, i), L.U(cur, i + 1)}, v3[3] = {L.V(cur, 0), L.V(cur, i), L.V(cur, i + 1)};
-                const float w3[3] = {L.P(cur, 0).w, L.P(cur, i).w, L.P(cur, i + 1).w};
-                write_mask_ext(&p.tris[gi + 1u], &p.materials[material], material, ts.area, u3, v3, w3);
-            }
-            bin_record_tiles(p, ts, gi | (masked ? CHORD_REC_MASKED : CHORD_REC_WIDE));
-        }
-    }
+    for (uint32_t k = block * CLIP_THREADS + threadIdx.x; k < n; k += blocks * CLIP_THREADS) clip_emit(p, L, p.clipTris[k], listShard);
 }
 
 #define CLIP_BLOCKS 64u
@@ -1435,44 +1532,7 @@
 #pragma unroll
         for (uint32_t st = 32u; st > 0u; st >>= 1) if (sStart[sh + st] <= k) sh += st;
         const uint32_t gi = __builtin_amdgcn_readfirstlane(p.largeList[(size_t)sh * p.largeCap + (k - sStart[sh])]);
-        const TriRec* __restrict__ r = &p.tris[gi];
-        TriSetup ts;
-#pragma unroll
-        for (int i = 0; i < 3; i++) { ts.X[i] = r->X[i]; ts.Y[i] = r->Y[i]; }
-        ts.payload = 0;
-        if (!tri_setup(ts, (r->twoSided & 1u) != 0, p.Wi, p.Hi)) continue;
-        const bool maskedRec = (r->twoSided & 4u) != 0u;
-        const int ea[3] = {1, 2, 0}, eb[3] = {2, 0, 1};
-        int64_t a[3], b[3], bias[3], dxe[3], dye[3];
-#pragma unroll
-        for (int i = 0; i < 3; i++) {
-            dxe[i] = (int64_t)(ts.X[eb[i]] - ts.X[ea[i]]); dye[i] = (int64_t)(ts.Y[eb[i]] - ts.Y[ea[i]]);
-            a[i] = -(int64_t)ts.s * dye[i]; b[i] = (int64_t)ts.s * dxe[i];
-            bias[i] = (a[i] > 0 || (a[i] == 0 && b[i] > 0)) ? 0 : -1;
-        }
-        const int32_t tx0 = ts.px0 >> TILE_SHIFT, tx1 = ts.px1 >> TILE_SHIFT;
-        const int32_t ty0 = ts.py0 >> TILE_SHIFT, ty1 = ts.py1 >> TILE_SHIFT;
-        const uint32_t tw = (uint32_t)(tx1 - tx0 + 1), nt = tw * (uint32_t)(ty1 - ty0 + 1);
-        for (uint32_t tb = 0; tb < nt; tb += 64u) {
-            const uint32_t t = tb + lane;
-            if (t >= nt) continue;
-            const int32_t tx = tx0 + (int32_t)(t % tw), ty = ty0 + (int32_t)(t / tw);
-            const int32_t rx0 = max(ts.px0, tx << TILE_SHIFT), rx1 = min(ts.px1, (tx << TILE_SHIFT) + TILE - 1);
-            const int32_t ry0 = max(ts.py0, ty << TILE_SHIFT), ry1 = min(ts.py1, (ty << TILE_SHIFT) + TILE - 1);
-            bool hit = owns_tile(p.shard, tx, ty);
-#pragma unroll
-            for (int i = 0; i < 3; i++) {
-                const int64_t cx = (int64_t)(a[i] > 0 ? rx1 : rx0) * 256 + 128, cy = (int64_t)(b[i] > 0 ? ry1 : ry0) * 256 + 128;
-                const int64_t E = (int64_t)ts.s * (dxe[i] * (cy - ts.Y[ea[i]]) - dye[i] * (cx - ts.X[ea[i]]));
-                hit = hit && !(E + bias[i] < 0);
-            }
-            if (hit) {
-                const uint32_t tile = (uint32_t)ty * p.tilesX + (uint32_t)tx;
-                const uint32_t slot = atomicAdd(&p.tileCount[(size_t)tile * TC_STRIDE], 1u);
-                bin_store(p, tile, slot, gi | (maskedRec ? CHORD_REC_MASKED : CHORD_REC_WIDE));
-                if (maskedRec) p.tileCount[(size_t)tile * TC_STRIDE + TC_MASKED] = 1u;
-            }
-        }
+        bin_large_record(p, gi, lane, p.Wi, p.Hi);
     }
 }
 
@@ -2797,6 +2857,8 @@
     p.tilesX = c->tilesX; p.tilesY = c->tilesY;
     p.clipTris = c->dClipTris + (size_t)pass * (c->clipTriCap / 2); p.clipTriCap = c->clipTriCap / 2; p.pass = pass;
     p.largeList = c->dLargeList + (size_t)pass * (c->largeCap / 2); p.largeCap = c->largeCap / 2 / CHORD_LIST_SHARDS;
+    static const int setupBinsMode = [] { const char* e = getenv("CHORDVIS_SETUP_BINS"); return e ? atoi(e) : 1; }();
+    p.setupBins = (setupBinsMode >= 2 || (setupBinsMode == 1 && pass >= 1u)) ? 1u : 0u;
     p.counters = c->dCounters;
     p.clearTiles = clearTiles ? 1u : 0u;
     p.depthOnly = c->depthOnly ? 1u : 0u; p.depthClamp = c->depthClamp ? 1u : 0u;
@@ -2860,7 +2922,7 @@
     if (c->anyMasked) CHORD_LAUNCH(c, raster_setup_kernel<true>, dim3(blocks), dim3(256), 0, c->stream, p);
     else              CHORD_LAUNCH(c, raster_setup_kernel<false>, dim3(blocks), dim3(256), 0, c->stream, p);
     stamp(c, S_R_CLUSTER);
-    CHORD_LAUNCH(c, raster_clip_and_bin_large_kernel, dim3(CLIP_BLOCKS + (uint32_t)c->numCUs * 4u), dim3(256), 0, c->stream, p);
+    if (!p.setupBins) CHORD_LAUNCH(c, raster_clip_and_bin_large_kernel, dim3(CLIP_BLOCKS + (uint32_t)c->numCUs * 4u), dim3(256), 0, c->stream, p);
     p.orderKept = 0u;
     p.heavyHint = nullptr;
     bool makeOrder = true;
```
